# jianzongwu/betrayed-by-captions

Hardware: NVIDIA B200
Metric: decoder_head_images_per_sec_1024 (higher is better)
Workload: dtype bf16

## Files before the change

### betrayed-by-captions_b200/csrc/attention_tc.cu

```cuda
#include <cstdio>
#include <cuda_fp16.h>
#include "kernels.h"
#include "tc_ptx.cuh"
#include "tc_state.h"

namespace cgg {

namespace {

constexpr int AT_THREADS = 64 + 512;
constexpr int AT_KT = 128;
constexpr int AT_STAGES = 4;
constexpr int AT_KV_TILE_BYTES = AT_KT * 64;
constexpr int AT_STAGE_BYTES = 4 * AT_KV_TILE_BYTES;
constexpr int AT_Q_BYTES = 128 * 64;
constexpr int AT_P_BYTES = 128 * AT_KT * 2;
constexpr float LOG2E = 1.4426950408889634f;

struct AttnP {
  const float* q; float* out; __nv_bfloat16* out_bf16;
  const uint32_t* bitmap; const uint8_t* all_masked; const uint8_t* live;
  int Q, K, heads, W32, ntiles, nqt;
  int trace;
  int has_r, r_col0, r_lo_off;
  int out_hl;
  int dbg;
};


__device__ __forceinline__ void store_attn_out(const AttnP& p, int b, int qi, int h, int C, const float* o, float inv) {
  if (p.out) {
    float4* dst = reinterpret_cast<float4*>(p.out + ((long)b * p.Q + qi) * C + h * 32);
#pragma unroll
    for (int i = 0; i < 8; ++i)
      dst[i] = make_float4(o[4 * i] * inv, o[4 * i + 1] * inv, o[4 * i + 2] * inv, o[4 * i + 3] * inv);
  }
  if (p.out_bf16) {
    const long ld = p.out_hl == 1 ? 2 * C : C;
    uint4* dst = reinterpret_cast<uint4*>(p.out_bf16 + ((long)b * p.Q + qi) * ld + h * 32);
    uint4* dst_lo = reinterpret_cast<uint4*>(p.out_bf16 + ((long)b * p.Q + qi) * ld + C + h * 32);
#pragma unroll
    for (int i = 0; i < 4; ++i) {
      uint4 pk, pl;
      uint32_t* w = reinterpret_cast<uint32_t*>(&pk);
      uint32_t* wl = reinterpret_cast<uint32_t*>(&pl);
#pragma unroll
      for (int j = 0; j < 4; ++j) {
        const float a0 = o[8 * i + 2 * j] * inv, a1 = o[8 * i + 2 * j + 1] * inv;
        if (p.out_hl == 2) {
          const __half2 h2 = __floats2half2_rn(a0, a1);
          w[j] = *reinterpret_cast<const uint32_t*>(&h2);
        } else {
          __nv_bfloat162 v2 = __floats2bfloat162_rn(a0, a1);
          w[j] = *reinterpret_cast<uint32_t*>(&v2);
          const float2 back = __bfloat1622float2(v2);
          __nv_bfloat162 l2 = __floats2bfloat162_rn(a0 - back.x, a1 - back.y);
          wl[j] = *reinterpret_cast<uint32_t*>(&l2);
        }
      }
      dst[i] = pk;
      if (p.out_hl == 1) dst_lo[i] = pl;
    }
  }
}

__device__ __forceinline__ void tmem_ld32(uint32_t taddr, float* v) {
  uint32_t r[32];
  asm volatile(
      "tcgen05.ld.sync.aligned.32x32b.x32.b32 {%0, %1, %2, %3, %4, %5, %6, %7, %8, %9, %10, %11, %12, %13, %14, %15, "
      "%16, %17, %18, %19, %20, %21, %22, %23, %24, %25, %26, %27, %28, %29, %30, %31}, [%32];"
      : "=r"(r[0]), "=r"(r[1]), "=r"(r[2]), "=r"(r[3]), "=r"(r[4]), "=r"(r[5]), "=r"(r[6]), "=r"(r[7]), "=r"(r[8]),
        "=r"(r[9]), "=r"(r[10]), "=r"(r[11]), "=r"(r[12]), "=r"(r[13]), "=r"(r[14]), "=r"(r[15]), "=r"(r[16]),
        "=r"(r[17]), "=r"(r[18]), "=r"(r[19]), "=r"(r[20]), "=r"(r[21]), "=r"(r[22]), "=r"(r[23]), "=r"(r[24]),
        "=r"(r[25]), "=r"(r[26]), "=r"(r[27]), "=r"(r[28]), "=r"(r[29]), "=r"(r[30]), "=r"(r[31])
      : "r"(taddr));
  asm volatile("tcgen05.wait::ld.sync.aligned;" ::: "memory");
#pragma unroll
  for (int i = 0; i < 32; ++i) v[i] = __uint_as_float(r[i]);
}

__device__ __forceinline__ float fast_exp2(float x) {
  float y;
  asm("ex2.approx.ftz.f32 %0, %1;" : "=f"(y) : "f"(x));
  return y;
}

__device__ __forceinline__ uint64_t umma_desc(uint32_t addr, uint32_t lbo, uint32_t sbo, uint32_t layout) {
  return (uint64_t)((addr >> 4) & 0x3FFFu) | ((uint64_t)((lbo >> 4) & 0x3FFFu) << 16) |
         ((uint64_t)((sbo >> 4) & 0x3FFFu) << 32) | (1ull << 46) | ((uint64_t)layout << 61);
}

__device__ __forceinline__ void fence_async_smem() { asm volatile("fence.proxy.async.shared::cta;" ::: "memory"); }

__device__ __forceinline__ int next_live(const uint8_t* live, int t, int n) {
  while (t < n && !live[t]) ++t;
  return t;
}

__device__ long long g_at_trace[64];
#ifdef CGG_AT_TRACING
#define AT_TRACE(ti, slot)                                                                                   \
  do {                                                                                                       \
    if (p.trace && blockIdx.x == 0 && blockIdx.y == 0 && (ti) >= 16 && (ti) < 24) g_at_trace[((ti) - 16) * 8 + (slot)] = clock64(); \
  } while (0)
#define AT_TRACE_W(ti, slot) do { if (warp == p.trace && lane == 0) AT_TRACE(ti, slot); } while (0)
#else
#define AT_TRACE(ti, slot) do { } while (0)
#define AT_TRACE_W(ti, slot) do { } while (0)
#endif

__global__ void __launch_bounds__(AT_THREADS, 1)
attention_tc_kernel(const __grid_constant__ CUtensorMap tmK, const __grid_constant__ CUtensorMap tmV,
                    const __grid_constant__ CUtensorMap tmR, const __grid_constant__ AttnP p) {
  extern __shared__ uint8_t smem_raw[];
  uint8_t* smem = reinterpret_cast<uint8_t*>((reinterpret_cast<uintptr_t>(smem_raw) + 1023) & ~(uintptr_t)1023);
  uint8_t* sQ = smem;
  uint8_t* sP = sQ + AT_Q_BYTES;
  uint8_t* sKV = sP + 2 * AT_P_BYTES;
  uint8_t* sLive = sKV + AT_STAGES * AT_STAGE_BYTES;
  uint64_t* bars = reinterpret_cast<uint64_t*>(sLive + 512);
  uint64_t* kv_full = bars;
  uint64_t* kv_empty = kv_full + AT_STAGES;
  uint64_t* step = kv_empty + AT_STAGES;
  uint64_t* p_full = step + 2;
  uint32_t* tmem_slot = reinterpret_cast<uint32_t*>(p_full + 2);

  const int warp = threadIdx.x >> 5, lane = threadIdx.x & 31;
  const int h = blockIdx.x % p.heads, qt = blockIdx.x / p.heads, b = blockIdx.y;
  const uint8_t* live = sLive;
  const int C = p.heads * 32;

  if (warp == 0 && lane == 0) {
    ptx::prefetch_tmap(&tmK);
    ptx::prefetch_tmap(&tmV);
    if (p.has_r) ptx::prefetch_tmap(&tmR);
    for (int i = 0; i < AT_STAGES; ++i) { ptx::mbar_init(&kv_full[i], 1); ptx::mbar_init(&kv_empty[i], 1); }
    for (int i = 0; i < 2; ++i) { ptx::mbar_init(&step[i], 1); ptx::mbar_init(&p_full[i], 512); }
    ptx::fence_mbar_init();
  }
  if (warp == 1) {
    ptx::tmem_alloc(tmem_slot, 512);
    ptx::tmem_relinquish();
  }
  ptx::grid_dep_launch();
  ptx::grid_dep_wait();
  {
    const int q0 = qt * 128, nrows = min(128, p.Q - q0);
    bool all_live = p.bitmap == nullptr;
    if (!all_live && p.all_masked)
      for (int r = lane; r < nrows; r += 32) all_live = all_live || p.all_masked[(long)b * p.Q + q0 + r] != 0;
    all_live = __any_sync(0xffffffffu, all_live);
    for (int t = warp; t < p.ntiles; t += AT_THREADS / 32) {
      bool any = all_live;
      if (!all_live) {
        for (int r = lane; r < nrows; r += 32) {
          const uint32_t* brow = p.bitmap + ((long)b * p.Q + q0 + r) * p.W32;
#pragma unroll
          for (int w = 0; w < 4; ++w) {
            const int widx = t * 4 + w, k0 = t * AT_KT + w * 32;
            if (widx < p.W32 && k0 < p.K) {
              const uint32_t valid = (k0 + 32 > p.K) ? ((1u << (p.K - k0)) - 1u) : 0xffffffffu;
              any = any || ((~__ldg(brow + widx)) & valid) != 0u;
            }
          }
        }
      }
      any = __any_sync(0xffffffffu, any);
      if (lane == 0) sLive[t] = any ? 1 : 0;
    }
  }
  if (warp >= 2 && warp < 6) {
    const int row = (warp & 3) * 32 + lane, qi = qt * 128 + row;
    float qv[32];
    if (qi < p.Q) {
      const float4* src = reinterpret_cast<const float4*>(p.q + ((long)b * p.Q + qi) * C + h * 32);
#pragma unroll
      for (int i = 0; i < 8; ++i) {
        const float4 x = __ldg(src + i);
        qv[4 * i] = x.x; qv[4 * i + 1] = x.y; qv[4 * i + 2] = x.z; qv[4 * i + 3] = x.w;
      }
    } else {
#pragma unroll
      for (int i = 0; i < 32; ++i) qv[i] = 0.f;
    }
#pragma unroll
    for (int c = 0; c < 4; ++c) {
      uint4 pk;
      uint32_t* w = reinterpret_cast<uint32_t*>(&pk);
#pragma unroll
      for (int j = 0; j < 4; ++j) {
        __nv_bfloat162 v2 = __floats2bfloat162_rn(qv[8 * c + 2 * j], qv[8 * c + 2 * j + 1]);
        w[j] = *reinterpret_cast<uint32_t*>(&v2);
      }
      *reinterpret_cast<uint4*>(sQ + (row >> 3) * 512 + c * 128 + (row & 7) * 16) = pk;
    }
    fence_async_smem();
  }
  ptx::tc_fence_before();
  __syncthreads();
  ptx::tc_fence_after();
  const uint32_t tmem_base = *tmem_slot;
  const uint32_t tmem_S = tmem_base;
  const uint32_t tmem_O = tmem_base + 256;

  if (warp == 0) {
    if (lane == 0) {
      int it = 0;
      for (int t = next_live(live, 0, p.ntiles); t < p.ntiles; t = next_live(live, t + 1, p.ntiles), ++it) {
        const int s = it % AT_STAGES;
        ptx::mbar_wait(&kv_empty[s], ((uint32_t)(it / AT_STAGES) & 1u) ^ 1u);
        ptx::mbar_expect_tx(&kv_full[s], (p.has_r ? (p.has_r > 1 ? 4 : 3) : 2) * AT_KV_TILE_BYTES);
        uint8_t* st = sKV + s * AT_STAGE_BYTES;
        if (p.has_r) {
          ptx::tma_load_2d(st + 2 * AT_KV_TILE_BYTES, &tmR, &kv_full[s], p.r_col0 + h * 32, t * AT_KT);
          if (p.has_r > 1) ptx::tma_load_2d(st + 3 * AT_KV_TILE_BYTES, &tmR, &kv_full[s], p.r_lo_off + p.r_col0 + h * 32, t * AT_KT);
        }
        ptx::tma_load_3d(st, &tmK, &kv_full[s], h * 32, t * AT_KT, b);
        ptx::tma_load_3d(st + AT_KV_TILE_BYTES, &tmV, &kv_full[s], h * 32, t * AT_KT, b);
      }
    }
  } else if (warp == 1) {
    const uint32_t idesc_s = ptx::umma_idesc_bf16(128, AT_KT, false, false);
    const uint32_t idesc_o = ptx::umma_idesc_bf16(128, 32, false, true);
    int n_live = 0;
    for (int t = 0; t < p.ntiles; ++t) n_live += live[t] ? 1 : 0;
    const uint64_t qd0 = umma_desc(ptx::smem_u32(sQ), 128, 512, 0);
    const uint64_t kd0 = umma_desc(ptx::smem_u32(sKV), 16, 512, 4);
    const uint64_t vd0 = umma_desc(ptx::smem_u32(sKV + AT_KV_TILE_BYTES), 1024, 512, 4);
    const uint64_t pd0 = umma_desc(ptx::smem_u32(sP), 128, 2048, 0);
    auto wait_kv = [&](int j) {
      ptx::mbar_wait(&kv_full[j % AT_STAGES], (uint32_t)(j / AT_STAGES) & 1u);
      ptx::tc_fence_after();
    };
    auto issue_qk = [&](int j) {
      const uint64_t kd = kd0 + (uint64_t)((j % AT_STAGES) * (AT_STAGE_BYTES >> 4));
      const uint32_t d = tmem_S + (uint32_t)((j & 1) * 128);
#pragma unroll
      for (int k = 0; k < 2; ++k) ptx::mma_bf16_ss(d, qd0 + (uint64_t)(k * 16), kd + (uint64_t)(k * 2), idesc_s, k);
      if (p.has_r) {
#pragma unroll
        for (int k = 0; k < 4; ++k)
          if (k < 2 || p.has_r > 1)
            ptx::mma_bf16_ss(d, qd0 + (uint64_t)((k & 1) * 16),
                             kd + (uint64_t)((((2 + (k >> 1)) * AT_KV_TILE_BYTES) >> 4) + (k & 1) * 2), idesc_s, 1u);
      }
    };
    for (int j = 0; j < 2 && j < n_live; ++j) {
      wait_kv(j);
      if (ptx::elect_one()) { issue_qk(j); ptx::mma_commit(&step[j]); }
      __syncwarp();
    }
    for (int j = 0; j < n_live; ++j) {
      const int s = j % AT_STAGES;
      ptx::mbar_wait(&p_full[j & 1], (uint32_t)(j >> 1) & 1u);
      if (j + 2 < n_live) wait_kv(j + 2);
      ptx::tc_fence_after();
      if (lane == 0) AT_TRACE(j, 0);
      if (ptx::elect_one()) {
        const uint64_t pd = pd0 + (uint64_t)((j & 1) * (AT_P_BYTES >> 4));
        const uint64_t vd = vd0 + (uint64_t)(s * (AT_STAGE_BYTES >> 4));
#pragma unroll
        for (int cq = 0; cq < 4; ++cq) {
#pragma unroll
          for (int k = 0; k < 2; ++k)
            ptx::mma_bf16_ss(tmem_O + (uint32_t)(((j & 1) * 4 + cq) * 32), pd + (uint64_t)((cq * 512 + k * 256) >> 4),
                             vd + (uint64_t)((cq * 2048 + k * 1024) >> 4), idesc_o, k);
        }
        if (j + 2 < n_live) issue_qk(j + 2);
        ptx::mma_commit(&step[j & 1]);
      }
      __syncwarp();
      if (lane == 0) AT_TRACE(j, 2);
    }
  } else {
    const int quarter = warp & 3;
    const int cq = (warp - 2) >> 2;
    const int row = quarter * 32 + lane, qi = qt * 128 + row;
    const bool row_ok = qi < p.Q;
    const uint32_t lane_off = (uint32_t)(quarter * 32) << 16;
    const bool ignore_mask = !row_ok || p.bitmap == nullptr || (p.all_masked && p.all_masked[(long)b * p.Q + qi]);
    const uint32_t* brow = p.bitmap ? p.bitmap + ((long)b * p.Q + (row_ok ? qi : 0)) * p.W32 : nullptr;
    float m_run = -INFINITY, l_run = 0.f;
    float o[32];
#pragma unroll
    for (int i = 0; i < 32; ++i) o[i] = 0.f;
    auto fold_o = [&](int pb, float scale) {
      float ov[32];
      tmem_ld32(tmem_O + (uint32_t)((pb * 4 + cq) * 32) + lane_off, ov);
      if (__all_sync(0xffffffffu, scale == 1.f)) {
#pragma unroll
        for (int i = 0; i < 32; ++i) o[i] += ov[i];
      } else {
#pragma unroll
        for (int i = 0; i < 32; ++i) o[i] = (o[i] + ov[i]) * scale;
      }
    };
    auto load_mask = [&](int t) -> uint32_t {
      const int widx = t * 4 + cq;
      uint32_t word = 0u;
      if (!ignore_mask && widx < p.W32) word = __ldg(brow + widx);
      const int k0 = t * AT_KT + cq * 32;
      if (k0 + 32 > p.K) word |= (k0 >= p.K) ? 0xffffffffu : ~((1u << (p.K - k0)) - 1u);
      return word;
    };
    int it = 0;
    uint32_t mw_next = 0u;
    {
      const int t0 = next_live(live, 0, p.ntiles);
      if (t0 < p.ntiles) mw_next = load_mask(t0);
    }
    for (int t = next_live(live, 0, p.ntiles); t < p.ntiles; ++it) {
      const int buf = it & 1;
      const int t_next = next_live(live, t + 1, p.ntiles);
      const uint32_t mw = mw_next;
      if (t_next < p.ntiles) mw_next = load_mask(t_next);
      ptx::mbar_wait(&step[buf], (uint32_t)(it >> 1) & 1u);
      ptx::tc_fence_after();
      AT_TRACE_W(it, 3);
      float v[32];
      tmem_ld32(tmem_S + (uint32_t)(buf * 128 + cq * 32) + lane_off, v);
      AT_TRACE_W(it, 4);
      float mx = -INFINITY;
#pragma unroll
      for (int i = 0; i < 32; ++i) {
        if ((mw >> i) & 1u) v[i] = -INFINITY;
        mx = fmaxf(mx, v[i]);
      }
      const float m_new = fmaxf(m_run, mx);
      const float scale = (m_new == -INFINITY) ? 1.f : fast_exp2((m_run - m_new) * LOG2E);
      const float mneg = (m_new == -INFINITY) ? 0.f : -m_new * LOG2E;
      m_run = m_new;
      uint8_t* prow = sP + buf * AT_P_BYTES + (row >> 3) * 2048 + (row & 7) * 16 + cq * 512;
      float psum = 0.f;
#pragma unroll
      for (int g = 0; g < 4; ++g) {
        uint4 pk;
        uint32_t* w = reinterpret_cast<uint32_t*>(&pk);
#pragma unroll
        for (int j = 0; j < 4; ++j) {
          const int i0 = g * 8 + 2 * j;
          const float e0 = fast_exp2(fmaf(v[i0], LOG2E, mneg)), e1 = fast_exp2(fmaf(v[i0 + 1], LOG2E, mneg));
          __nv_bfloat162 v2 = __floats2bfloat162_rn(e0, e1);
          w[j] = *reinterpret_cast<uint32_t*>(&v2);
          psum += e0 + e1;
        }
        *reinterpret_cast<uint4*>(prow + g * 128) = pk;
      }
      l_run = l_run * scale + psum;
      fence_async_smem();
      ptx::tc_fence_before();
      ptx::mbar_arrive(&p_full[buf]);
      AT_TRACE_W(it, 5);
      if (it > 0) {
        ptx::mbar_wait(&step[(it - 1) & 1], (uint32_t)(((it - 1) >> 1) + 1) & 1u);
        ptx::tc_fence_after();
        if (warp == 2 && lane == 0) ptx::mbar_arrive(&kv_empty[(it - 1) % AT_STAGES]);
        AT_TRACE_W(it, 6);
        fold_o((it - 1) & 1, scale);
      }
      AT_TRACE_W(it, 7);
      t = t_next;
    }
    if (it > 0) {
      ptx::mbar_wait(&step[(it - 1) & 1], (uint32_t)(((it - 1) >> 1) + 1) & 1u);
      ptx::tc_fence_after();
      fold_o((it - 1) & 1, 1.f);
    }
    float* xch = reinterpret_cast<float*>(sP);
    if (cq > 0) {
      float* dst = xch + ((cq - 1) * 128 + row) * 35;
      dst[0] = m_run;
      dst[1] = l_run;
#pragma unroll
      for (int i = 0; i < 32; ++i) dst[2 + i] = o[i];
    }
    asm volatile("bar.sync 1, 512;" ::: "memory");
    const int hf = cq;
    if (cq == 0) {
      float m = m_run;
#pragma unroll
      for (int c2 = 0; c2 < 3; ++c2) m = fmaxf(m, xch[(c2 * 128 + row) * 35]);
      const float a0 = (m_run == -INFINITY) ? 0.f : fast_exp2((m_run - m) * LOG2E);
      l_run *= a0;
#pragma unroll
      for (int i = 0; i < 32; ++i) o[i] *= a0;
#pragma unroll
      for (int c2 = 0; c2 < 3; ++c2) {
        const float* src = xch + (c2 * 128 + row) * 35;
        const float m1 = src[0];
        const float a1 = (m1 == -INFINITY) ? 0.f : fast_exp2((m1 - m) * LOG2E);
        l_run += src[1] * a1;
#pragma unroll
        for (int i = 0; i < 32; ++i) o[i] += src[2 + i] * a1;
      }
    }
    if (row_ok && hf == 0) store_attn_out(p, b, qi, h, C, o, l_run > 0.f ? 1.0f / l_run : 0.f);
  }
  ptx::tc_fence_before();
  __syncthreads();
  if (warp == 1) {
    __syncwarp();
    ptx::tmem_dealloc(tmem_base, 512);
  }
}


__device__ __forceinline__ void tmem_st32(uint32_t taddr, const float* v) {
  asm volatile(
      "tcgen05.st.sync.aligned.32x32b.x32.b32 [%0], {%1, %2, %3, %4, %5, %6, %7, %8, %9, %10, %11, %12, %13, %14, %15, %16, "
      "%17, %18, %19, %20, %21, %22, %23, %24, %25, %26, %27, %28, %29, %30, %31, %32};"
      ::"r"(taddr), "r"(__float_as_uint(v[0])), "r"(__float_as_uint(v[1])), "r"(__float_as_uint(v[2])), "r"(__float_as_uint(v[3])),
        "r"(__float_as_uint(v[4])), "r"(__float_as_uint(v[5])), "r"(__float_as_uint(v[6])), "r"(__float_as_uint(v[7])),
        "r"(__float_as_uint(v[8])), "r"(__float_as_uint(v[9])), "r"(__float_as_uint(v[10])), "r"(__float_as_uint(v[11])),
        "r"(__float_as_uint(v[12])), "r"(__float_as_uint(v[13])), "r"(__float_as_uint(v[14])), "r"(__float_as_uint(v[15])),
        "r"(__float_as_uint(v[16])), "r"(__float_as_uint(v[17])), "r"(__float_as_uint(v[18])), "r"(__float_as_uint(v[19])),
        "r"(__float_as_uint(v[20])), "r"(__float_as_uint(v[21])), "r"(__float_as_uint(v[22])), "r"(__float_as_uint(v[23])),
        "r"(__float_as_uint(v[24])), "r"(__float_as_uint(v[25])), "r"(__float_as_uint(v[26])), "r"(__float_as_uint(v[27])),
        "r"(__float_as_uint(v[28])), "r"(__float_as_uint(v[29])), "r"(__float_as_uint(v[30])), "r"(__float_as_uint(v[31]))
      : "memory");
  asm volatile("tcgen05.wait::st.sync.aligned;" ::: "memory");
}
__device__ __forceinline__ void tmem_st16(uint32_t taddr, const uint32_t* r) {
  asm volatile(
      "tcgen05.st.sync.aligned.32x32b.x16.b32 [%0], {%1, %2, %3, %4, %5, %6, %7, %8, %9, %10, %11, %12, %13, %14, %15, %16};"
      ::"r"(taddr), "r"(r[0]), "r"(r[1]), "r"(r[2]), "r"(r[3]), "r"(r[4]), "r"(r[5]), "r"(r[6]), "r"(r[7]), "r"(r[8]), "r"(r[9]),
        "r"(r[10]), "r"(r[11]), "r"(r[12]), "r"(r[13]), "r"(r[14]), "r"(r[15])
      : "memory");
  asm volatile("tcgen05.wait::st.sync.aligned;" ::: "memory");
}
__device__ __forceinline__ void mma_bf16_ts(uint32_t d_tmem, uint32_t a_tmem, uint64_t bdesc, uint32_t idesc, uint32_t accumulate) {
  asm volatile(
      "{\n\t.reg .pred p;\n\tsetp.ne.b32 p, %4, 0;\n\t"
      "tcgen05.mma.cta_group::1.kind::f16 [%0], [%1], %2, %3, p;\n\t}\n"
      ::"r"(d_tmem), "r"(a_tmem), "l"(bdesc), "r"(idesc), "r"(accumulate)
      : "memory");
}

constexpr float AT2_TAU = 8.0f;

__global__ void __launch_bounds__(AT_THREADS, 1)
attention_tc2_kernel(const __grid_constant__ CUtensorMap tmK, const __grid_constant__ CUtensorMap tmV,
                     const __grid_constant__ CUtensorMap tmR, const __grid_constant__ AttnP p) {
  extern __shared__ uint8_t smem_raw[];
  uint8_t* smem = reinterpret_cast<uint8_t*>((reinterpret_cast<uintptr_t>(smem_raw) + 1023) & ~(uintptr_t)1023);
  uint8_t* sQ = smem;
  uint8_t* sX = sQ + AT_Q_BYTES;
  uint8_t* sKV = sX + 2 * AT_P_BYTES;
  uint8_t* sLive = sKV + AT_STAGES * AT_STAGE_BYTES;
  uint64_t* bars = reinterpret_cast<uint64_t*>(sLive + 512);
  uint64_t* kv_full = bars;
  uint64_t* kv_empty = kv_full + AT_STAGES;
  uint64_t* step = kv_empty + AT_STAGES;
  uint64_t* p_full = step + 2;
  uint32_t* tmem_slot = reinterpret_cast<uint32_t*>(p_full + 2);

  const int warp = threadIdx.x >> 5, lane = threadIdx.x & 31;
  const int h = blockIdx.x % p.heads, qt = blockIdx.x / p.heads, b = blockIdx.y;
  const uint8_t* live = sLive;
  const int C = p.heads * 32;

  if (warp == 0 && lane == 0) {
    ptx::prefetch_tmap(&tmK);
    ptx::prefetch_tmap(&tmV);
    if (p.has_r) ptx::prefetch_tmap(&tmR);
    for (int i = 0; i < AT_STAGES; ++i) { ptx::mbar_init(&kv_full[i], 1); ptx::mbar_init(&kv_empty[i], 1); }
    for (int i = 0; i < 2; ++i) { ptx::mbar_init(&step[i], 1); ptx::mbar_init(&p_full[i], 512); }
    ptx::fence_mbar_init();
  }
  if (warp == 1) {
    ptx::tmem_alloc(tmem_slot, 512);
    ptx::tmem_relinquish();
  }
  ptx::grid_dep_launch();
  ptx::grid_dep_wait();
  {
    const int q0 = qt * 128, nrows = min(128, p.Q - q0);
    bool all_live = p.bitmap == nullptr;
    if (!all_live && p.all_masked)
      for (int r = lane; r < nrows; r += 32) all_live = all_live || p.all_masked[(long)b * p.Q + q0 + r] != 0;
    all_live = __any_sync(0xffffffffu, all_live);
    for (int t = warp; t < p.ntiles; t += AT_THREADS / 32) {
      bool any = all_live;
      if (!all_live) {
        for (int r = lane; r < nrows; r += 32) {
          const uint32_t* brow = p.bitmap + ((long)b * p.Q + q0 + r) * p.W32;
#pragma unroll
          for (int w = 0; w < 4; ++w) {
            const int widx = t * 4 + w, k0 = t * AT_KT + w * 32;
            if (widx < p.W32 && k0 < p.K) {
              const uint32_t valid = (k0 + 32 > p.K) ? ((1u << (p.K - k0)) - 1u) : 0xffffffffu;
              any = any || ((~__ldg(brow + widx)) & valid) != 0u;
            }
          }
        }
      }
      any = __any_sync(0xffffffffu, any);
      if (lane == 0) sLive[t] = any ? 1 : 0;
    }
  }
  if (warp >= 2 && warp < 6) {
    const int row = (warp & 3) * 32 + lane, qi = qt * 128 + row;
    float qv[32];
    if (qi < p.Q) {
      const float4* src = reinterpret_cast<const float4*>(p.q + ((long)b * p.Q + qi) * C + h * 32);
#pragma unroll
      for (int i = 0; i < 8; ++i) {
        const float4 x = __ldg(src + i);
        qv[4 * i] = x.x; qv[4 * i + 1] = x.y; qv[4 * i + 2] = x.z; qv[4 * i + 3] = x.w;
      }
    } else {
#pragma unroll
      for (int i = 0; i < 32; ++i) qv[i] = 0.f;
    }
#pragma unroll
    for (int c = 0; c < 4; ++c) {
      uint4 pk;
      uint32_t* w = reinterpret_cast<uint32_t*>(&pk);
#pragma unroll
      for (int j = 0; j < 4; ++j) {
        __nv_bfloat162 v2 = __floats2bfloat162_rn(qv[8 * c + 2 * j], qv[8 * c + 2 * j + 1]);
        w[j] = *reinterpret_cast<uint32_t*>(&v2);
      }
      *reinterpret_cast<uint4*>(sQ + (row >> 3) * 512 + c * 128 + (row & 7) * 16) = pk;
    }
    fence_async_smem();
  }
  ptx::tc_fence_before();
  __syncthreads();
  ptx::tc_fence_after();
  const uint32_t tmem_base = *tmem_slot;
  const uint32_t tmem_S = tmem_base;
  const uint32_t tmem_P = tmem_base + 256;
  const uint32_t tmem_O = tmem_base + 384;

  if (warp == 0) {
    if (lane == 0) {
      int it = 0;
      for (int t = next_live(live, 0, p.ntiles); t < p.ntiles; t = next_live(live, t + 1, p.ntiles), ++it) {
        const int s = it % AT_STAGES;
        ptx::mbar_wait(&kv_empty[s], ((uint32_t)(it / AT_STAGES) & 1u) ^ 1u);
        ptx::mbar_expect_tx(&kv_full[s], (p.has_r ? (p.has_r > 1 ? 4 : 3) : 2) * AT_KV_TILE_BYTES);
        uint8_t* st = sKV + s * AT_STAGE_BYTES;
        if (p.has_r) {
          ptx::tma_load_2d(st + 2 * AT_KV_TILE_BYTES, &tmR, &kv_full[s], p.r_col0 + h * 32, t * AT_KT);
          if (p.has_r > 1) ptx::tma_load_2d(st + 3 * AT_KV_TILE_BYTES, &tmR, &kv_full[s], p.r_lo_off + p.r_col0 + h * 32, t * AT_KT);
        }
        ptx::tma_load_3d(st, &tmK, &kv_full[s], h * 32, t * AT_KT, b);
        ptx::tma_load_3d(st + AT_KV_TILE_BYTES, &tmV, &kv_full[s], h * 32, t * AT_KT, b);
      }
    }
  } else if (warp == 1) {
    const uint32_t idesc_s = ptx::umma_idesc_bf16(128, AT_KT, false, false);
    const uint32_t idesc_o = ptx::umma_idesc_bf16(128, 32, false, true);
    int n_live = 0;
    for (int t = 0; t < p.ntiles; ++t) n_live += live[t] ? 1 : 0;
    const uint64_t qd0 = umma_desc(ptx::smem_u32(sQ), 128, 512, 0);
    const uint64_t kd0 = umma_desc(ptx::smem_u32(sKV), 16, 512, 4);
    const uint64_t vd0 = umma_desc(ptx::smem_u32(sKV + AT_KV_TILE_BYTES), 1024, 512, 4);
    auto wait_kv = [&](int j) {
      ptx::mbar_wait(&kv_full[j % AT_STAGES], (uint32_t)(j / AT_STAGES) & 1u);
      ptx::tc_fence_after();
    };
    auto issue_qk = [&](int j) {
      const uint64_t kd = kd0 + (uint64_t)((j % AT_STAGES) * (AT_STAGE_BYTES >> 4));
      const uint32_t d = tmem_S + (uint32_t)((j & 1) * 128);
#pragma unroll
      for (int k = 0; k < 2; ++k) ptx::mma_bf16_ss(d, qd0 + (uint64_t)(k * 16), kd + (uint64_t)(k * 2), idesc_s, k);
      if (p.has_r) {
#pragma unroll
        for (int k = 0; k < 4; ++k)
          if (k < 2 || p.has_r > 1)
            ptx::mma_bf16_ss(d, qd0 + (uint64_t)((k & 1) * 16),
                             kd + (uint64_t)((((2 + (k >> 1)) * AT_KV_TILE_BYTES) >> 4) + (k & 1) * 2), idesc_s, 1u);
      }
    };
    for (int j = 0; j < 2 && j < n_live; ++j) {
      wait_kv(j);
      if (ptx::elect_one()) { issue_qk(j); ptx::mma_commit(&step[j]); }
      __syncwarp();
    }
    for (int j = 0; j < n_live; ++j) {
      const int s = j % AT_STAGES;
      ptx::mbar_wait(&p_full[j & 1], (uint32_t)(j >> 1) & 1u);
      if (lane == 0) AT_TRACE(j, 0);
      if (j + 2 < n_live) wait_kv(j + 2);
      ptx::tc_fence_after();
      if (lane == 0) AT_TRACE(j, 1);
      if (ptx::elect_one()) {
        const uint64_t vd = vd0 + (uint64_t)(s * (AT_STAGE_BYTES >> 4));
        const uint32_t pa = tmem_P + (uint32_t)((j & 1) * 64);
#pragma unroll
        for (int cq = 0; cq < 4; ++cq) {
          if (p.dbg & 2) break;
#pragma unroll
          for (int k = 0; k < 2; ++k)
            mma_bf16_ts(tmem_O + (uint32_t)(cq * 32), pa + (uint32_t)(cq * 16 + k * 8),
                        vd + (uint64_t)((cq * 2048 + k * 1024) >> 4), idesc_o, (j > 0 || k > 0) ? 1u : 0u);
        }
        if (j + 2 < n_live) issue_qk(j + 2);
        ptx::mma_commit(&step[j & 1]);
      }
      __syncwarp();
      if (lane == 0) AT_TRACE(j, 2);
    }
  } else {
    const int quarter = warp & 3;
    const int cq = (warp - 2) >> 2;
    const int row = quarter * 32 + lane, qi = qt * 128 + row;
    const bool row_ok = qi < p.Q;
    const uint32_t lane_off = (uint32_t)(quarter * 32) << 16;
    const bool ignore_mask = !row_ok || p.bitmap == nullptr || (p.all_masked && p.all_masked[(long)b * p.Q + qi]);
    const uint32_t* brow = p.bitmap ? p.bitmap + ((long)b * p.Q + (row_ok ? qi : 0)) * p.W32 : nullptr;
    const uint32_t taddr_o = tmem_O + (uint32_t)(cq * 32) + lane_off;
    float m_ref = -INFINITY, l_run = 0.f;
    auto load_mask = [&](int t) -> uint32_t {
      const int widx = t * 4 + cq;
      uint32_t word = 0u;
      if (!ignore_mask && widx < p.W32) word = __ldg(brow + widx);
      const int k0 = t * AT_KT + cq * 32;
      if (k0 + 32 > p.K) word |= (k0 >= p.K) ? 0xffffffffu : ~((1u << (p.K - k0)) - 1u);
      return word;
    };
    int it = 0;
    uint32_t mw_next = 0u;
    {
      const int t0 = next_live(live, 0, p.ntiles);
      if (t0 < p.ntiles) mw_next = load_mask(t0);
    }
    for (int t = next_live(live, 0, p.ntiles); t < p.ntiles; ++it) {
      const int buf = it & 1;
      const int t_next = next_live(live, t + 1, p.ntiles);
      const uint32_t mw = mw_next;
      if (t_next < p.ntiles) mw_next = load_mask(t_next);
      ptx::mbar_wait(&step[buf], (uint32_t)(it >> 1) & 1u);
      ptx::tc_fence_after();
      AT_TRACE_W(it, 3);
      float v[32];
      tmem_ld32(tmem_S + (uint32_t)(buf * 128 + cq * 32) + lane_off, v);
      AT_TRACE_W(it, 4);
      float mx = -INFINITY;
#pragma unroll
      for (int i = 0; i < 32; ++i) {
        if ((mw >> i) & 1u) v[i] = -INFINITY;
        mx = fmaxf(mx, v[i]);
      }
      mx *= LOG2E;
      const bool move = mx > m_ref + AT2_TAU;
      const bool fix = move && m_ref != -INFINITY;
      if (__any_sync(0xffffffffu, fix)) {
        ptx::mbar_wait(&step[(it - 1) & 1], (uint32_t)(((it - 1) >> 1) + 1) & 1u);
        ptx::tc_fence_after();
        const float sc = fix ? fast_exp2(m_ref - mx) : 1.f;
        float ov[32];
        tmem_ld32(taddr_o, ov);
#pragma unroll
        for (int i = 0; i < 32; ++i) ov[i] *= sc;
        tmem_st32(taddr_o, ov);
        l_run *= sc;
      }
      if (move) m_ref = mx;
      AT_TRACE_W(it, 5);
      const float mneg = (m_ref == -INFINITY) ? 0.f : -m_ref;
      uint32_t pk[16];
      float psum = 0.f;
#pragma unroll
      for (int j = 0; j < 16; ++j) {
        float e0, e1;
        if (p.dbg & 4) { e0 = fmaf(v[2 * j], LOG2E, mneg); e1 = fmaf(v[2 * j + 1], LOG2E, mneg); }
        else { e0 = fast_exp2(fmaf(v[2 * j], LOG2E, mneg)); e1 = fast_exp2(fmaf(v[2 * j + 1], LOG2E, mneg)); }
        __nv_bfloat162 v2 = __floats2bfloat162_rn(e0, e1);
        pk[j] = *reinterpret_cast<uint32_t*>(&v2);
        psum += e0 + e1;
      }
      l_run += psum;
      AT_TRACE_W(it, 6);
      tmem_st16(tmem_P + (uint32_t)(buf * 64 + cq * 16) + lane_off, pk);
      ptx::tc_fence_before();
      ptx::mbar_arrive(&p_full[buf]);
      AT_TRACE_W(it, 7);
      if (it > 0 && warp == 2) {
        ptx::mbar_wait(&step[(it - 1) & 1], (uint32_t)(((it - 1) >> 1) + 1) & 1u);
        if (lane == 0) ptx::mbar_arrive(&kv_empty[(it - 1) % AT_STAGES]);
      }
      t = t_next;
    }
    float o[32];
    if (it > 0) {
      ptx::mbar_wait(&step[(it - 1) & 1], (uint32_t)(((it - 1) >> 1) + 1) & 1u);
      ptx::tc_fence_after();
      tmem_ld32(taddr_o, o);
    } else {
#pragma unroll
      for (int i = 0; i < 32; ++i) o[i] = 0.f;
    }
    float* xch = reinterpret_cast<float*>(sX);
    if (cq > 0) {
      float* dst = xch + ((cq - 1) * 128 + row) * 35;
      dst[0] = m_ref;
      dst[1] = l_run;
#pragma unroll
      for (int i = 0; i < 32; ++i) dst[2 + i] = o[i];
    }
    asm volatile("bar.sync 1, 512;" ::: "memory");
    if (cq == 0) {
      float m = m_ref;
#pragma unroll
      for (int c2 = 0; c2 < 3; ++c2) m = fmaxf(m, xch[(c2 * 128 + row) * 35]);
      const float a0 = (m_ref == -INFINITY) ? 0.f : fast_exp2(m_ref - m);
      l_run *= a0;
#pragma unroll
      for (int i = 0; i < 32; ++i) o[i] = (m_ref == -INFINITY) ? 0.f : o[i] * a0;
#pragma unroll
      for (int c2 = 0; c2 < 3; ++c2) {
        const float* src = xch + (c2 * 128 + row) * 35;
        const float m1 = src[0];
        if (m1 != -INFINITY) {
          const float a1 = fast_exp2(m1 - m);
          l_run += src[1] * a1;
#pragma unroll
          for (int i = 0; i < 32; ++i) o[i] += src[2 + i] * a1;
        }
      }
      if (row_ok) store_attn_out(p, b, qi, h, C, o, l_run > 0.f ? 1.0f / l_run : 0.f);
    }
  }
  ptx::tc_fence_before();
  __syncthreads();
  if (warp == 1) {
    __syncwarp();
    ptx::tmem_dealloc(tmem_base, 512);
  }
}

constexpr int AT3_STAGES = 6;

__global__ void __launch_bounds__(AT_THREADS, 1)
attention_tc3_kernel(const __grid_constant__ CUtensorMap tmK, const __grid_constant__ CUtensorMap tmV,
                     const __grid_constant__ CUtensorMap tmR, const __grid_constant__ AttnP p) {
  extern __shared__ uint8_t smem_raw[];
  uint8_t* smem = reinterpret_cast<uint8_t*>((reinterpret_cast<uintptr_t>(smem_raw) + 1023) & ~(uintptr_t)1023);
  uint8_t* sQ = smem;
  uint8_t* sKV = sQ + AT_Q_BYTES;
  uint8_t* sX = sKV;
  uint8_t* sLive = sKV + AT3_STAGES * AT_STAGE_BYTES;
  uint64_t* bars = reinterpret_cast<uint64_t*>(sLive + 512);
  uint64_t* kv_full = bars;
  uint64_t* kv_empty = kv_full + AT3_STAGES;
  uint64_t* step = kv_empty + AT3_STAGES;
  uint64_t* p_full = step + 3;
  uint32_t* tmem_slot = reinterpret_cast<uint32_t*>(p_full + 3);

  const int warp = threadIdx.x >> 5, lane = threadIdx.x & 31;
  const int h = blockIdx.x % p.heads, qt = blockIdx.x / p.heads, b = blockIdx.y;
  const uint8_t* live = sLive;
  const int C = p.heads * 32;

  if (warp == 0 && lane == 0) {
    ptx::prefetch_tmap(&tmK);
    ptx::prefetch_tmap(&tmV);
    if (p.has_r) ptx::prefetch_tmap(&tmR);
    for (int i = 0; i < AT3_STAGES; ++i) { ptx::mbar_init(&kv_full[i], 1); ptx::mbar_init(&kv_empty[i], 1); }
    for (int i = 0; i < 3; ++i) { ptx::mbar_init(&step[i], 1); ptx::mbar_init(&p_full[i], 512); }
    ptx::fence_mbar_init();
  }
  if (warp == 1) {
    ptx::tmem_alloc(tmem_slot, 512);
    ptx::tmem_relinquish();
  }
  ptx::grid_dep_launch();
  ptx::grid_dep_wait();
  {
    const int q0 = qt * 128, nrows = min(128, p.Q - q0);
    bool all_live = p.bitmap == nullptr;
    if (!all_live && p.all_masked)
      for (int r = lane; r < nrows; r += 32) all_live = all_live || p.all_masked[(long)b * p.Q + q0 + r] != 0;
    all_live = __any_sync(0xffffffffu, all_live);
    for (int t = warp; t < p.ntiles; t += AT_THREADS / 32) {
      bool any = all_live;
      if (!all_live) {
        for (int r = lane; r < nrows; r += 32) {
          const uint32_t* brow = p.bitmap + ((long)b * p.Q + q0 + r) * p.W32;
#pragma unroll
          for (int w = 0; w < 4; ++w) {
            const int widx = t * 4 + w, k0 = t * AT_KT + w * 32;
            if (widx < p.W32 && k0 < p.K) {
              const uint32_t valid = (k0 + 32 > p.K) ? ((1u << (p.K - k0)) - 1u) : 0xffffffffu;
              any = any || ((~__ldg(brow + widx)) & valid) != 0u;
            }
          }
        }
      }
      any = __any_sync(0xffffffffu, any);
      if (lane == 0) sLive[t] = any ? 1 : 0;
    }
  }
  if (warp >= 2 && warp < 6) {
    const int row = (warp & 3) * 32 + lane, qi = qt * 128 + row;
    float qv[32];
    if (qi < p.Q) {
      const float4* src = reinterpret_cast<const float4*>(p.q + ((long)b * p.Q + qi) * C + h * 32);
#pragma unroll
      for (int i = 0; i < 8; ++i) {
        const float4 x = __ldg(src + i);
        qv[4 * i] = x.x; qv[4 * i + 1] = x.y; qv[4 * i + 2] = x.z; qv[4 * i + 3] = x.w;
      }
    } else {
#pragma unroll
      for (int i = 0; i < 32; ++i) qv[i] = 0.f;
    }
#pragma unroll
    for (int c = 0; c < 4; ++c) {
      uint4 pk;
      uint32_t* w = reinterpret_cast<uint32_t*>(&pk);
#pragma unroll
      for (int j = 0; j < 4; ++j) {
        __nv_bfloat162 v2 = __floats2bfloat162_rn(qv[8 * c + 2 * j], qv[8 * c + 2 * j + 1]);
        w[j] = *reinterpret_cast<uint32_t*>(&v2);
      }
      *reinterpret_cast<uint4*>(sQ + (row >> 3) * 512 + c * 128 + (row & 7) * 16) = pk;
    }
    fence_async_smem();
  }
  ptx::tc_fence_before();
  __syncthreads();
  ptx::tc_fence_after();
  const uint32_t tmem_base = *tmem_slot;
  const uint32_t tmem_S = tmem_base;
  const uint32_t tmem_O = tmem_base + 384;

  if (warp == 0) {
    if (lane == 0) {
      int it = 0;
      for (int t = next_live(live, 0, p.ntiles); t < p.ntiles; t = next_live(live, t + 1, p.ntiles), ++it) {
        const int s = it % AT3_STAGES;
        ptx::mbar_wait(&kv_empty[s], ((uint32_t)(it / AT3_STAGES) & 1u) ^ 1u);
        ptx::mbar_expect_tx(&kv_full[s], (p.has_r ? (p.has_r > 1 ? 4 : 3) : 2) * AT_KV_TILE_BYTES);
        uint8_t* st = sKV + s * AT_STAGE_BYTES;
        if (p.has_r) {
          ptx::tma_load_2d(st + 2 * AT_KV_TILE_BYTES, &tmR, &kv_full[s], p.r_col0 + h * 32, t * AT_KT);
          if (p.has_r > 1) ptx::tma_load_2d(st + 3 * AT_KV_TILE_BYTES, &tmR, &kv_full[s], p.r_lo_off + p.r_col0 + h * 32, t * AT_KT);
        }
        ptx::tma_load_3d(st, &tmK, &kv_full[s], h * 32, t * AT_KT, b);
        ptx::tma_load_3d(st + AT_KV_TILE_BYTES, &tmV, &kv_full[s], h * 32, t * AT_KT, b);
      }
    }
  } else if (warp == 1) {
    const uint32_t idesc_s = ptx::umma_idesc_bf16(128, AT_KT, false, false);
    const uint32_t idesc_o = ptx::umma_idesc_bf16(128, 32, false, true);
    int n_live = 0;
    for (int t = 0; t < p.ntiles; ++t) n_live += live[t] ? 1 : 0;
    const uint64_t qd0 = umma_desc(ptx::smem_u32(sQ), 128, 512, 0);
    const uint64_t kd0 = umma_desc(ptx::smem_u32(sKV), 16, 512, 4);
    const uint64_t vd0 = umma_desc(ptx::smem_u32(sKV + AT_KV_TILE_BYTES), 1024, 512, 4);
    auto wait_kv = [&](int j) {
      ptx::mbar_wait(&kv_full[j % AT3_STAGES], (uint32_t)(j / AT3_STAGES) & 1u);
      ptx::tc_fence_after();
    };
    auto issue_qk = [&](int j) {
      const uint64_t kd = kd0 + (uint64_t)((j % AT3_STAGES) * (AT_STAGE_BYTES >> 4));
      const uint32_t d = tmem_S + (uint32_t)((j % 3) * 128);
#pragma unroll
      for (int k = 0; k < 2; ++k) ptx::mma_bf16_ss(d, qd0 + (uint64_t)(k * 16), kd + (uint64_t)(k * 2), idesc_s, k);
      if (p.has_r) {
#pragma unroll
        for (int k = 0; k < 4; ++k)
          if (k < 2 || p.has_r > 1)
            ptx::mma_bf16_ss(d, qd0 + (uint64_t)((k & 1) * 16),
                             kd + (uint64_t)((((2 + (k >> 1)) * AT_KV_TILE_BYTES) >> 4) + (k & 1) * 2), idesc_s, 1u);
      }
    };
    for (int j = 0; j < 3 && j < n_live; ++j) {
      wait_kv(j);
      if (ptx::elect_one()) { issue_qk(j); ptx::mma_commit(&step[j]); }
      __syncwarp();
    }
    for (int j = 0; j < n_live; ++j) {
      const int s = j % AT3_STAGES;
      ptx::mbar_wait(&p_full[j % 3], (uint32_t)(j / 3) & 1u);
      if (lane == 0) AT_TRACE(j, 0);
      if (j + 3 < n_live) wait_kv(j + 3);
      ptx::tc_fence_after();
      if (lane == 0) AT_TRACE(j, 1);
      if (ptx::elect_one()) {
        const uint64_t vd = vd0 + (uint64_t)(s * (AT_STAGE_BYTES >> 4));
        const uint32_t pa = tmem_S + (uint32_t)((j % 3) * 128);
#pragma unroll
        for (int cq = 0; cq < 4; ++cq) {
          if (p.dbg & 2) break;
#pragma unroll
          for (int k = 0; k < 2; ++k)
            mma_bf16_ts(tmem_O + (uint32_t)(cq * 32), pa + (uint32_t)(cq * 32 + k * 8),
                        vd + (uint64_t)((cq * 2048 + k * 1024) >> 4), idesc_o, (j > 0 || k > 0) ? 1u : 0u);
        }
        if (j + 3 < n_live) issue_qk(j + 3);
        ptx::mma_commit(&step[j % 3]);
      }
      __syncwarp();
      if (lane == 0) AT_TRACE(j, 2);
    }
  } else {
    const int quarter = warp & 3;
    const int cq = (warp - 2) >> 2;
    const int row = quarter * 32 + lane, qi = qt * 128 + row;
    const bool row_ok = qi < p.Q;
    const uint32_t lane_off = (uint32_t)(quarter * 32) << 16;
    const bool ignore_mask = !row_ok || p.bitmap == nullptr || (p.all_masked && p.all_masked[(long)b * p.Q + qi]);
    const uint32_t* brow = p.bitmap ? p.bitmap + ((long)b * p.Q + (row_ok ? qi : 0)) * p.W32 : nullptr;
    const uint32_t taddr_o = tmem_O + (uint32_t)(cq * 32) + lane_off;
    float m_ref = -INFINITY, l_run = 0.f;
    auto load_mask = [&](int t) -> uint32_t {
      const int widx = t * 4 + cq;
      uint32_t word = 0u;
      if (!ignore_mask && widx < p.W32) word = __ldg(brow + widx);
      const int k0 = t * AT_KT + cq * 32;
      if (k0 + 32 > p.K) word |= (k0 >= p.K) ? 0xffffffffu : ~((1u << (p.K - k0)) - 1u);
      return word;
    };
    int it = 0;
    uint32_t mw_next = 0u;
    {
      const int t0 = next_live(live, 0, p.ntiles);
      if (t0 < p.ntiles) mw_next = load_mask(t0);
    }
    for (int t = next_live(live, 0, p.ntiles); t < p.ntiles; ++it) {
      const int buf = it % 3;
      const int t_next = next_live(live, t + 1, p.ntiles);
      const uint32_t mw = mw_next;
      if (t_next < p.ntiles) mw_next = load_mask(t_next);
      ptx::mbar_wait(&step[buf], (uint32_t)(it / 3) & 1u);
      ptx::tc_fence_after();
      AT_TRACE_W(it, 3);
      float v[32];
      tmem_ld32(tmem_S + (uint32_t)(buf * 128 + cq * 32) + lane_off, v);
      AT_TRACE_W(it, 4);
      float mx = -INFINITY;
#pragma unroll
      for (int i = 0; i < 32; ++i) {
        if ((mw >> i) & 1u) v[i] = -INFINITY;
        mx = fmaxf(mx, v[i]);
      }
      mx *= LOG2E;
      const bool move = mx > m_ref + AT2_TAU;
      const bool fix = move && m_ref != -INFINITY;
      if (__any_sync(0xffffffffu, fix)) {
        ptx::mbar_wait(&step[(it - 1) % 3], (uint32_t)(((it - 1) / 3) + 1) & 1u);
        ptx::tc_fence_after();
        const float sc = fix ? fast_exp2(m_ref - mx) : 1.f;
        float ov[32];
        tmem_ld32(taddr_o, ov);
#pragma unroll
        for (int i = 0; i < 32; ++i) ov[i] *= sc;
        tmem_st32(taddr_o, ov);
        l_run *= sc;
      }
      if (move) m_ref = mx;
      AT_TRACE_W(it, 5);
      const float mneg = (m_ref == -INFINITY) ? 0.f : -m_ref;
      uint32_t pk[16];
      float psum = 0.f;
#pragma unroll
      for (int j = 0; j < 16; ++j) {
        float e0, e1;
        if (p.dbg & 4) { e0 = fmaf(v[2 * j], LOG2E, mneg); e1 = fmaf(v[2 * j + 1], LOG2E, mneg); }
        else { e0 = fast_exp2(fmaf(v[2 * j], LOG2E, mneg)); e1 = fast_exp2(fmaf(v[2 * j + 1], LOG2E, mneg)); }
        __nv_bfloat162 v2 = __floats2bfloat162_rn(e0, e1);
        pk[j] = *reinterpret_cast<uint32_t*>(&v2);
        psum += e0 + e1;
      }
      l_run += psum;
      AT_TRACE_W(it, 6);
      tmem_st16(tmem_S + (uint32_t)(buf * 128 + cq * 32) + lane_off, pk);
      ptx::tc_fence_before();
      ptx::mbar_arrive(&p_full[buf]);
      AT_TRACE_W(it, 7);
      if (it > 0 && warp == 2) {
        ptx::mbar_wait(&step[(it - 1) % 3], (uint32_t)(((it - 1) / 3) + 1) & 1u);
        if (lane == 0) ptx::mbar_arrive(&kv_empty[(it - 1) % AT3_STAGES]);
      }
      t = t_next;
    }
    float o[32];
    if (it > 0) {
      ptx::mbar_wait(&step[(it - 1) % 3], (uint32_t)(((it - 1) / 3) + 1) & 1u);
      ptx::tc_fence_after();
      tmem_ld32(taddr_o, o);
    } else {
#pragma unroll
      for (int i = 0; i < 32; ++i) o[i] = 0.f;
    }
    asm volatile("bar.sync 1, 512;" ::: "memory");
    float* xch = reinterpret_cast<float*>(sX);
    if (cq > 0) {
      float* dst = xch + ((cq - 1) * 128 + row) * 35;
      dst[0] = m_ref;
      dst[1] = l_run;
#pragma unroll
      for (int i = 0; i < 32; ++i) dst[2 + i] = o[i];
    }
    asm volatile("bar.sync 1, 512;" ::: "memory");
    if (cq == 0) {
      float m = m_ref;
#pragma unroll
      for (int c2 = 0; c2 < 3; ++c2) m = fmaxf(m, xch[(c2 * 128 + row) * 35]);
      const float a0 = (m_ref == -INFINITY) ? 0.f : fast_exp2(m_ref - m);
      l_run *= a0;
#pragma unroll
      for (int i = 0; i < 32; ++i) o[i] = (m_ref == -INFINITY) ? 0.f : o[i] * a0;
#pragma unroll
      for (int c2 = 0; c2 < 3; ++c2) {
        const float* src = xch + (c2 * 128 + row) * 35;
        const float m1 = src[0];
        if (m1 != -INFINITY) {
          const float a1 = fast_exp2(m1 - m);
          l_run += src[1] * a1;
#pragma unroll
          for (int i = 0; i < 32; ++i) o[i] += src[2 + i] * a1;
        }
      }
      if (row_ok) store_attn_out(p, b, qi, h, C, o, l_run > 0.f ? 1.0f / l_run : 0.f);
    }
  }
  ptx::tc_fence_before();
  __syncthreads();
  if (warp == 1) {
    __syncwarp();
    ptx::tmem_dealloc(tmem_base, 512);
  }
}

int make_map_kv(TcState* t, CUtensorMap* m, const void* base, int K, long kv_stride, long kv_bstride, int B, int C) {
  if ((kv_stride * 2) % 16 != 0 || (kv_bstride * 2) % 16 != 0 || (reinterpret_cast<uintptr_t>(base) & 15))
    return tc_fail(t, CGG_ERR_UNSUPPORTED, "K/V rows must be 16-byte aligned");
  cuuint64_t dims[3] = {(cuuint64_t)C, (cuuint64_t)K, (cuuint64_t)B};
  cuuint64_t strides[2] = {(cuuint64_t)kv_stride * 2, (cuuint64_t)kv_bstride * 2};
  cuuint32_t box[3] = {32, AT_KT, 1};
  cuuint32_t es[3] = {1, 1, 1};
  CUresult r = t->encode(m, CU_TENSOR_MAP_DATA_TYPE_BFLOAT16, 3, const_cast<void*>(base), dims, strides, box, es,
                         CU_TENSOR_MAP_INTERLEAVE_NONE, CU_TENSOR_MAP_SWIZZLE_64B, CU_TENSOR_MAP_L2_PROMOTION_L2_128B,
                         CU_TENSOR_MAP_FLOAT_OOB_FILL_NONE);
  if (r != CUDA_SUCCESS) return tc_fail(t, CGG_ERR_CUDA, "cuTensorMapEncodeTiled(KV) failed: " + std::to_string((int)r));
  return CGG_OK;
}

}

int tc_attention(TcState* t, int batch, int num_keys, const float* q, const void* k, const void* v, long kv_stride,
                 long kv_bstride, const uint32_t* bitmap, const uint8_t* all_masked, float* out, __nv_bfloat16* out_bf16,
                 cudaStream_t s, const void* r_table, long r_cols, int r_col0, int out_mode) {
  const int Q = t->cfg.num_queries, heads = t->cfg.num_heads, C = t->cfg.embed_dim;
  const int ntiles = (num_keys + AT_KT - 1) / AT_KT, nqt = (Q + 127) / 128;
  CUtensorMap mK, mV;
  int st = make_map_kv(t, &mK, k, num_keys, kv_stride, kv_bstride, batch, C);
  if (st != CGG_OK) return st;
  st = make_map_kv(t, &mV, v, num_keys, kv_stride, kv_bstride, batch, C);
  if (st != CGG_OK) return st;
  CUtensorMap mR = mK;
  if (r_table) {
    cuuint64_t dims[2] = {(cuuint64_t)r_cols, (cuuint64_t)num_keys};
    cuuint64_t strides[1] = {(cuuint64_t)r_cols * 2};
    cuuint32_t box[2] = {32, AT_KT};
    cuuint32_t es[2] = {1, 1};
    CUresult r = t->encode(&mR, CU_TENSOR_MAP_DATA_TYPE_BFLOAT16, 2, const_cast<void*>(r_table), dims, strides, box, es,
                           CU_TENSOR_MAP_INTERLEAVE_NONE, CU_TENSOR_MAP_SWIZZLE_64B, CU_TENSOR_MAP_L2_PROMOTION_L2_128B,
                           CU_TENSOR_MAP_FLOAT_OOB_FILL_NONE);
    if (r != CUDA_SUCCESS) return tc_fail(t, CGG_ERR_CUDA, "cuTensorMapEncodeTiled(R) failed: " + std::to_string((int)r));
  }
  const int W32 = (num_keys + 31) / 32;
  AttnP p;
  p.q = q; p.out = out; p.out_bf16 = out_bf16; p.bitmap = bitmap; p.all_masked = all_masked; p.live = nullptr;
  p.Q = Q; p.K = num_keys; p.heads = heads; p.W32 = W32; p.ntiles = ntiles; p.nqt = nqt;
  p.has_r = r_table ? 2 : 0;
  p.r_col0 = r_col0; p.r_lo_off = (int)(r_cols / 2);
  p.out_hl = out_mode;
#ifdef CGG_AT_TRACING
  static const int at_dbg = getenv("CGG_AT_DBG") ? atoi(getenv("CGG_AT_DBG")) : 0;
  p.dbg = at_dbg;
  if (at_dbg & 1) p.has_r = 0;
#else
  p.dbg = 0;
#endif
  if (ntiles > 512) return tc_fail(t, CGG_ERR_BAD_SHAPE, "more than 512 key tiles");
  const size_t smem = 1024 + AT_Q_BYTES + 2 * AT_P_BYTES + AT_STAGES * AT_STAGE_BYTES + 512 + (2 * AT_STAGES + 4) * 8 + 16;
  if (!t->attn_attr_set) {
    TCU(cudaFuncSetAttribute(attention_tc_kernel, cudaFuncAttributeMaxDynamicSharedMemorySize, (int)smem));
    TCU(cudaFuncSetAttribute(attention_tc2_kernel, cudaFuncAttributeMaxDynamicSharedMemorySize, (int)smem));
    TCU(cudaFuncSetAttribute(attention_tc3_kernel, cudaFuncAttributeMaxDynamicSharedMemorySize, 227 * 1024));
    t->attn_attr_set = true;
  }
  static const bool trace = getenv("CGG_AT_TRACE") != nullptr;
  p.trace = trace ? atoi(getenv("CGG_AT_TRACE")) : 0;
  static const int use_v1 = getenv("CGG_ATTN_V1") ? atoi(getenv("CGG_ATTN_V1")) : 0;
  static const int use_v3 = getenv("CGG_ATTN_V3") ? atoi(getenv("CGG_ATTN_V3")) : 1;
  const size_t smem3 = 1024 + AT_Q_BYTES + AT3_STAGES * AT_STAGE_BYTES + 512 + (2 * AT3_STAGES + 6) * 8 + 16;
  if (use_v1) TCU(launch_pdl(attention_tc_kernel, dim3(heads * nqt, batch), dim3(AT_THREADS), smem, s, mK, mV, mR, p));
  else if (use_v3) TCU(launch_pdl(attention_tc3_kernel, dim3(heads * nqt, batch), dim3(AT_THREADS), smem3, s, mK, mV, mR, p));
  else TCU(launch_pdl(attention_tc2_kernel, dim3(heads * nqt, batch), dim3(AT_THREADS), smem, s, mK, mV, mR, p));
  count_launch();
  TCU(cudaGetLastError());
  if (trace && ntiles >= 24) {
    cudaStreamSynchronize(s);
    long long tr[64];
    cudaMemcpyFromSymbol(tr, g_at_trace, sizeof(tr));
    fprintf(stderr, "[attention trace] K=%d cycles rel. to tile 16: mma(P ready, PV committed, QK(j+2) committed) softmax(S ready, S loaded, P arrived, O(j-1) ready, folded)\n", num_keys);
    for (int i = 0; i < 8; ++i) {
      fprintf(stderr, "  j=%d:", 16 + i);
      for (int j = 0; j < 8; ++j) fprintf(stderr, " %7lld", tr[i * 8 + j] - tr[0]);
      fprintf(stderr, "\n");
    }
  }
  return CGG_OK;
}

}
```

Baseline: 6497.

## Consolidate masked attention into one kernel with staged masks and precomputed live tiles

Removes the v1/v2 attention variants and keeps a single v3-style kernel. The per-CTA live-tile scan moves into a separate small pre-kernel that writes live flags to global memory. The producer warp now loads the per-row mask words alongside each K/V stage into shared memory, so softmax warps no longer issue their own global mask loads. Other changes: stages go from 4 to 6, TMEM loads and stores are split into issue and wait so they overlap with math, and the max and sum reductions use trees and packed f32x2 math. The cost is an extra kernel launch and a more complex producer path with 32-arrival barriers.

New measurement: 6716 (median of 6 runs). 3.4% higher.

```diff
diff --git a/betrayed-by-captions_b200/csrc/attention_tc.cu b/betrayed-by-captions_b200/csrc/attention_tc.cu
--- a/betrayed-by-captions_b200/csrc/attention_tc.cu
+++ b/betrayed-by-captions_b200/csrc/attention_tc.cu
@@ -10,21 +10,26 @@
 
 constexpr int AT_THREADS = 64 + 512;
 constexpr int AT_KT = 128;
-constexpr int AT_STAGES = 4;
+constexpr int AT_STAGES = 6;
 constexpr int AT_KV_TILE_BYTES = AT_KT * 64;
 constexpr int AT_STAGE_BYTES = 4 * AT_KV_TILE_BYTES;
+constexpr int AT_MASK_BYTES = 128 * 4 * 4;
 constexpr int AT_Q_BYTES = 128 * 64;
-constexpr int AT_P_BYTES = 128 * AT_KT * 2;
+constexpr int AT_MAX_TILES = 512;
 constexpr float LOG2E = 1.4426950408889634f;
+constexpr float AT_TAU = 8.0f;
+constexpr size_t AT_SMEM = 1024 + AT_Q_BYTES + AT_STAGES * (AT_STAGE_BYTES + AT_MASK_BYTES) + AT_MAX_TILES +
+                           (2 * AT_STAGES + 6) * 8 + 16;
+static_assert(AT_SMEM <= 227 * 1024, "attention stage budget");
 
 struct AttnP {
   const float* q; float* out; __nv_bfloat16* out_bf16;
-  const uint32_t* bitmap; const uint8_t* all_masked; const uint8_t* live;
+  const uint32_t* bitmap; const uint8_t* all_masked;
+  const uint8_t* live;
   int Q, K, heads, W32, ntiles, nqt;
   int trace;
   int has_r, r_col0, r_lo_off;
   int out_hl;
-  int dbg;
 };
 
 
@@ -97,6 +102,60 @@
   return t;
 }
 
+__device__ __forceinline__ void tmem_ld32_issue(uint32_t taddr, uint32_t* r) {
+  asm volatile(
+      "tcgen05.ld.sync.aligned.32x32b.x32.b32 {%0, %1, %2, %3, %4, %5, %6, %7, %8, %9, %10, %11, %12, %13, %14, %15, "
+      "%16, %17, %18, %19, %20, %21, %22, %23, %24, %25, %26, %27, %28, %29, %30, %31}, [%32];"
+      : "=r"(r[0]), "=r"(r[1]), "=r"(r[2]), "=r"(r[3]), "=r"(r[4]), "=r"(r[5]), "=r"(r[6]), "=r"(r[7]), "=r"(r[8]),
+        "=r"(r[9]), "=r"(r[10]), "=r"(r[11]), "=r"(r[12]), "=r"(r[13]), "=r"(r[14]), "=r"(r[15]), "=r"(r[16]),
+        "=r"(r[17]), "=r"(r[18]), "=r"(r[19]), "=r"(r[20]), "=r"(r[21]), "=r"(r[22]), "=r"(r[23]), "=r"(r[24]),
+        "=r"(r[25]), "=r"(r[26]), "=r"(r[27]), "=r"(r[28]), "=r"(r[29]), "=r"(r[30]), "=r"(r[31])
+      : "r"(taddr));
+}
+__device__ __forceinline__ void tmem_ld32_wait(uint32_t* r) {
+  asm volatile("tcgen05.wait::ld.sync.aligned;"
+               : "+r"(r[0]), "+r"(r[1]), "+r"(r[2]), "+r"(r[3]), "+r"(r[4]), "+r"(r[5]), "+r"(r[6]), "+r"(r[7]),
+                 "+r"(r[8]), "+r"(r[9]), "+r"(r[10]), "+r"(r[11]), "+r"(r[12]), "+r"(r[13]), "+r"(r[14]), "+r"(r[15]),
+                 "+r"(r[16]), "+r"(r[17]), "+r"(r[18]), "+r"(r[19]), "+r"(r[20]), "+r"(r[21]), "+r"(r[22]),
+                 "+r"(r[23]), "+r"(r[24]), "+r"(r[25]), "+r"(r[26]), "+r"(r[27]), "+r"(r[28]), "+r"(r[29]),
+                 "+r"(r[30]), "+r"(r[31])
+               :: "memory");
+}
+__device__ __forceinline__ void tmem_st16_issue(uint32_t taddr, const uint32_t* r) {
+  asm volatile(
+      "tcgen05.st.sync.aligned.32x32b.x16.b32 [%0], {%1, %2, %3, %4, %5, %6, %7, %8, %9, %10, %11, %12, %13, %14, %15, %16};"
+      ::"r"(taddr), "r"(r[0]), "r"(r[1]), "r"(r[2]), "r"(r[3]), "r"(r[4]), "r"(r[5]), "r"(r[6]), "r"(r[7]), "r"(r[8]), "r"(r[9]),
+        "r"(r[10]), "r"(r[11]), "r"(r[12]), "r"(r[13]), "r"(r[14]), "r"(r[15])
+      : "memory");
+}
+__device__ __forceinline__ void tmem_st16_wait(uint32_t* r) {
+  asm volatile("tcgen05.wait::st.sync.aligned;"
+               : "+r"(r[0]), "+r"(r[1]), "+r"(r[2]), "+r"(r[3]), "+r"(r[4]), "+r"(r[5]), "+r"(r[6]), "+r"(r[7]),
+                 "+r"(r[8]), "+r"(r[9]), "+r"(r[10]), "+r"(r[11]), "+r"(r[12]), "+r"(r[13]), "+r"(r[14]), "+r"(r[15])
+               :: "memory");
+}
+
+__device__ __forceinline__ float2 fma2(float2 a, float2 b, float2 c) {
+  float2 d;
+  asm("{\n\t.reg .b64 ra, rb, rc, rd;\n\t"
+      "mov.b64 ra, {%2, %3};\n\tmov.b64 rb, {%4, %5};\n\tmov.b64 rc, {%6, %7};\n\t"
+      "fma.rn.f32x2 rd, ra, rb, rc;\n\tmov.b64 {%0, %1}, rd;\n\t}"
+      : "=f"(d.x), "=f"(d.y) : "f"(a.x), "f"(a.y), "f"(b.x), "f"(b.y), "f"(c.x), "f"(c.y));
+  return d;
+}
+__device__ __forceinline__ float2 add2(float2 a, float2 b) {
+  float2 d;
+  asm("{\n\t.reg .b64 ra, rb, rd;\n\t"
+      "mov.b64 ra, {%2, %3};\n\tmov.b64 rb, {%4, %5};\n\t"
+      "add.rn.f32x2 rd, ra, rb;\n\tmov.b64 {%0, %1}, rd;\n\t}"
+      : "=f"(d.x), "=f"(d.y) : "f"(a.x), "f"(a.y), "f"(b.x), "f"(b.y));
+  return d;
+}
+
+__device__ __forceinline__ void mbar_expect_tx_only(uint64_t* bar, uint32_t bytes) {
+  asm volatile("mbarrier.expect_tx.relaxed.cta.shared::cta.b64 [%0], %1;" ::"r"(ptx::smem_u32(bar)), "r"(bytes) : "memory");
+}
+
 __device__ long long g_at_trace[64];
 #ifdef CGG_AT_TRACING
 #define AT_TRACE(ti, slot)                                                                                   \
@@ -109,21 +168,58 @@
 #define AT_TRACE_W(ti, slot) do { } while (0)
 #endif
 
+__device__ __forceinline__ void mma_bf16_ts(uint32_t d_tmem, uint32_t a_tmem, uint64_t bdesc, uint32_t idesc, uint32_t accumulate) {
+  asm volatile(
+      "{\n\t.reg .pred p;\n\tsetp.ne.b32 p, %4, 0;\n\t"
+      "tcgen05.mma.cta_group::1.kind::f16 [%0], [%1], %2, %3, p;\n\t}\n"
+      ::"r"(d_tmem), "r"(a_tmem), "l"(bdesc), "r"(idesc), "r"(accumulate)
+      : "memory");
+}
+
+__global__ void __launch_bounds__(512) attention_live_kernel(const uint32_t* __restrict__ bitmap,
+                                                             const uint8_t* __restrict__ all_masked, int Q, int K,
+                                                             int W32, int ntiles, int nqt, uint8_t* __restrict__ live) {
+  __shared__ int s_tile[AT_MAX_TILES];
+  __shared__ int s_fallback;
+  const int qt = blockIdx.x, b = blockIdx.y, warp = threadIdx.x >> 5, lane = threadIdx.x & 31;
+  for (int t = threadIdx.x; t < ntiles; t += blockDim.x) s_tile[t] = 0;
+  if (threadIdx.x == 0) s_fallback = 0;
+  ptx::grid_dep_launch();
+  ptx::grid_dep_wait();
+  __syncthreads();
+  const int q0 = qt * 128, nrows = min(128, Q - q0);
+  for (int r = warp; r < nrows; r += blockDim.x / 32) {
+    const long row = (long)b * Q + q0 + r;
+    if (all_masked && all_masked[row]) { s_fallback = 1; continue; }
+    const uint32_t* brow = bitmap + row * W32;
+#pragma unroll 4
+    for (int w = lane; w < W32; w += 32) {
+      const int k0 = w * 32;
+      const uint32_t valid = (k0 + 32 > K) ? ((1u << (K - k0)) - 1u) : 0xffffffffu;
+      if ((~__ldg(brow + w)) & valid) s_tile[w >> 2] = 1;
+    }
+  }
+  __syncthreads();
+  for (int t = threadIdx.x; t < ntiles; t += blockDim.x)
+    live[((long)b * nqt + qt) * ntiles + t] = (s_fallback || s_tile[t]) ? 1 : 0;
+}
+
 __global__ void __launch_bounds__(AT_THREADS, 1)
-attention_tc_kernel(const __grid_constant__ CUtensorMap tmK, const __grid_constant__ CUtensorMap tmV,
-                    const __grid_constant__ CUtensorMap tmR, const __grid_constant__ AttnP p) {
+masked_attention_tc_kernel(const __grid_constant__ CUtensorMap tmK, const __grid_constant__ CUtensorMap tmV,
+                           const __grid_constant__ CUtensorMap tmR, const __grid_constant__ AttnP p) {
   extern __shared__ uint8_t smem_raw[];
   uint8_t* smem = reinterpret_cast<uint8_t*>((reinterpret_cast<uintptr_t>(smem_raw) + 1023) & ~(uintptr_t)1023);
   uint8_t* sQ = smem;
-  uint8_t* sP = sQ + AT_Q_BYTES;
-  uint8_t* sKV = sP + 2 * AT_P_BYTES;
-  uint8_t* sLive = sKV + AT_STAGES * AT_STAGE_BYTES;
-  uint64_t* bars = reinterpret_cast<uint64_t*>(sLive + 512);
+  uint8_t* sKV = sQ + AT_Q_BYTES;
+  uint8_t* sX = sKV;
+  uint32_t* sMask = reinterpret_cast<uint32_t*>(sKV + AT_STAGES * AT_STAGE_BYTES);
+  uint8_t* sLive = reinterpret_cast<uint8_t*>(sMask) + AT_STAGES * AT_MASK_BYTES;
+  uint64_t* bars = reinterpret_cast<uint64_t*>(sLive + AT_MAX_TILES);
   uint64_t* kv_full = bars;
   uint64_t* kv_empty = kv_full + AT_STAGES;
   uint64_t* step = kv_empty + AT_STAGES;
-  uint64_t* p_full = step + 2;
-  uint32_t* tmem_slot = reinterpret_cast<uint32_t*>(p_full + 2);
+  uint64_t* p_full = step + 3;
+  uint32_t* tmem_slot = reinterpret_cast<uint32_t*>(p_full + 3);
 
   const int warp = threadIdx.x >> 5, lane = threadIdx.x & 31;
   const int h = blockIdx.x % p.heads, qt = blockIdx.x / p.heads, b = blockIdx.y;
@@ -134,8 +230,8 @@
     ptx::prefetch_tmap(&tmK);
     ptx::prefetch_tmap(&tmV);
     if (p.has_r) ptx::prefetch_tmap(&tmR);
-    for (int i = 0; i < AT_STAGES; ++i) { ptx::mbar_init(&kv_full[i], 1); ptx::mbar_init(&kv_empty[i], 1); }
-    for (int i = 0; i < 2; ++i) { ptx::mbar_init(&step[i], 1); ptx::mbar_init(&p_full[i], 512); }
+    for (int i = 0; i < AT_STAGES; ++i) { ptx::mbar_init(&kv_full[i], 32); ptx::mbar_init(&kv_empty[i], 1); }
+    for (int i = 0; i < 3; ++i) { ptx::mbar_init(&step[i], 1); ptx::mbar_init(&p_full[i], 512); }
     ptx::fence_mbar_init();
   }
   if (warp == 1) {
@@ -145,29 +241,8 @@
   ptx::grid_dep_launch();
   ptx::grid_dep_wait();
   {
-    const int q0 = qt * 128, nrows = min(128, p.Q - q0);
-    bool all_live = p.bitmap == nullptr;
-    if (!all_live && p.all_masked)
-      for (int r = lane; r < nrows; r += 32) all_live = all_live || p.all_masked[(long)b * p.Q + q0 + r] != 0;
-    all_live = __any_sync(0xffffffffu, all_live);
-    for (int t = warp; t < p.ntiles; t += AT_THREADS / 32) {
-      bool any = all_live;
-      if (!all_live) {
-        for (int r = lane; r < nrows; r += 32) {
-          const uint32_t* brow = p.bitmap + ((long)b * p.Q + q0 + r) * p.W32;
-#pragma unroll
-          for (int w = 0; w < 4; ++w) {
-            const int widx = t * 4 + w, k0 = t * AT_KT + w * 32;
-            if (widx < p.W32 && k0 < p.K) {
-              const uint32_t valid = (k0 + 32 > p.K) ? ((1u << (p.K - k0)) - 1u) : 0xffffffffu;
-              any = any || ((~__ldg(brow + widx)) & valid) != 0u;
-            }
-          }
-        }
-      }
-      any = __any_sync(0xffffffffu, any);
-      if (lane == 0) sLive[t] = any ? 1 : 0;
-    }
+    const uint8_t* src = p.live ? p.live + ((long)b * p.nqt + qt) * p.ntiles : nullptr;
+    for (int t = threadIdx.x; t < p.ntiles; t += AT_THREADS) sLive[t] = src ? src[t] : 1;
   }
   if (warp >= 2 && warp < 6) {
     const int row = (warp & 3) * 32 + lane, qi = qt * 128 + row;
@@ -201,15 +276,24 @@
   ptx::tc_fence_after();
   const uint32_t tmem_base = *tmem_slot;
   const uint32_t tmem_S = tmem_base;
-  const uint32_t tmem_O = tmem_base + 256;
+  const uint32_t tmem_O = tmem_base + 384;
 
   if (warp == 0) {
-    if (lane == 0) {
-      int it = 0;
-      for (int t = next_live(live, 0, p.ntiles); t < p.ntiles; t = next_live(live, t + 1, p.ntiles), ++it) {
-        const int s = it % AT_STAGES;
-        ptx::mbar_wait(&kv_empty[s], ((uint32_t)(it / AT_STAGES) & 1u) ^ 1u);
-        ptx::mbar_expect_tx(&kv_full[s], (p.has_r ? (p.has_r > 1 ? 4 : 3) : 2) * AT_KV_TILE_BYTES);
+    const uint32_t* brow[4];
+#pragma unroll
+    for (int i = 0; i < 4; ++i) {
+      const int qi = qt * 128 + lane + 32 * i;
+      const bool use = p.bitmap && qi < p.Q && !(p.all_masked && p.all_masked[(long)b * p.Q + qi]);
+      brow[i] = use ? p.bitmap + ((long)b * p.Q + qi) * p.W32 : nullptr;
+    }
+    const bool vec = (p.W32 & 3) == 0 && (reinterpret_cast<uintptr_t>(p.bitmap) & 15) == 0;
+    const uint32_t tx_bytes = (p.has_r ? (p.has_r > 1 ? 4 : 3) : 2) * AT_KV_TILE_BYTES;
+    int it = 0;
+    for (int t = next_live(live, 0, p.ntiles); t < p.ntiles; t = next_live(live, t + 1, p.ntiles), ++it) {
+      const int s = it % AT_STAGES;
+      ptx::mbar_wait(&kv_empty[s], ((uint32_t)(it / AT_STAGES) & 1u) ^ 1u);
+      if (lane == 0) {
+        mbar_expect_tx_only(&kv_full[s], tx_bytes);
         uint8_t* st = sKV + s * AT_STAGE_BYTES;
         if (p.has_r) {
           ptx::tma_load_2d(st + 2 * AT_KV_TILE_BYTES, &tmR, &kv_full[s], p.r_col0 + h * 32, t * AT_KT);
@@ -218,336 +302,26 @@
         ptx::tma_load_3d(st, &tmK, &kv_full[s], h * 32, t * AT_KT, b);
         ptx::tma_load_3d(st + AT_KV_TILE_BYTES, &tmV, &kv_full[s], h * 32, t * AT_KT, b);
       }
-    }
-  } else if (warp == 1) {
-    const uint32_t idesc_s = ptx::umma_idesc_bf16(128, AT_KT, false, false);
-    const uint32_t idesc_o = ptx::umma_idesc_bf16(128, 32, false, true);
-    int n_live = 0;
-    for (int t = 0; t < p.ntiles; ++t) n_live += live[t] ? 1 : 0;
-    const uint64_t qd0 = umma_desc(ptx::smem_u32(sQ), 128, 512, 0);
-    const uint64_t kd0 = umma_desc(ptx::smem_u32(sKV), 16, 512, 4);
-    const uint64_t vd0 = umma_desc(ptx::smem_u32(sKV + AT_KV_TILE_BYTES), 1024, 512, 4);
-    const uint64_t pd0 = umma_desc(ptx::smem_u32(sP), 128, 2048, 0);
-    auto wait_kv = [&](int j) {
-      ptx::mbar_wait(&kv_full[j % AT_STAGES], (uint32_t)(j / AT_STAGES) & 1u);
-      ptx::tc_fence_after();
-    };
-    auto issue_qk = [&](int j) {
-      const uint64_t kd = kd0 + (uint64_t)((j % AT_STAGES) * (AT_STAGE_BYTES >> 4));
-      const uint32_t d = tmem_S + (uint32_t)((j & 1) * 128);
-#pragma unroll
-      for (int k = 0; k < 2; ++k) ptx::mma_bf16_ss(d, qd0 + (uint64_t)(k * 16), kd + (uint64_t)(k * 2), idesc_s, k);
-      if (p.has_r) {
-#pragma unroll
-        for (int k = 0; k < 4; ++k)
-          if (k < 2 || p.has_r > 1)
-            ptx::mma_bf16_ss(d, qd0 + (uint64_t)((k & 1) * 16),
-                             kd + (uint64_t)((((2 + (k >> 1)) * AT_KV_TILE_BYTES) >> 4) + (k & 1) * 2), idesc_s, 1u);
-      }
-    };
-    for (int j = 0; j < 2 && j < n_live; ++j) {
-      wait_kv(j);
-      if (ptx::elect_one()) { issue_qk(j); ptx::mma_commit(&step[j]); }
-      __syncwarp();
-    }
-    for (int j = 0; j < n_live; ++j) {
-      const int s = j % AT_STAGES;
-      ptx::mbar_wait(&p_full[j & 1], (uint32_t)(j >> 1) & 1u);
-      if (j + 2 < n_live) wait_kv(j + 2);
-      ptx::tc_fence_after();
-      if (lane == 0) AT_TRACE(j, 0);
-      if (ptx::elect_one()) {
-        const uint64_t pd = pd0 + (uint64_t)((j & 1) * (AT_P_BYTES >> 4));
-        const uint64_t vd = vd0 + (uint64_t)(s * (AT_STAGE_BYTES >> 4));
-#pragma unroll
-        for (int cq = 0; cq < 4; ++cq) {
-#pragma unroll
-          for (int k = 0; k < 2; ++k)
-            ptx::mma_bf16_ss(tmem_O + (uint32_t)(((j & 1) * 4 + cq) * 32), pd + (uint64_t)((cq * 512 + k * 256) >> 4),
-                             vd + (uint64_t)((cq * 2048 + k * 1024) >> 4), idesc_o, k);
+      uint32_t w[4][4];
+#pragma unroll
+      for (int i = 0; i < 4; ++i) {
+        if (brow[i] && vec) {
+          const uint4 x = __ldg(reinterpret_cast<const uint4*>(brow[i] + t * 4));
+          w[i][0] = x.x; w[i][1] = x.y; w[i][2] = x.z; w[i][3] = x.w;
+        } else {
+#pragma unroll
+          for (int c = 0; c < 4; ++c) w[i][c] = (brow[i] && t * 4 + c < p.W32) ? __ldg(brow[i] + t * 4 + c) : 0u;
         }
-        if (j + 2 < n_live) issue_qk(j + 2);
-        ptx::mma_commit(&step[j & 1]);
-      }
-      __syncwarp();
-      if (lane == 0) AT_TRACE(j, 2);
-    }
-  } else {
-    const int quarter = warp & 3;
-    const int cq = (warp - 2) >> 2;
-    const int row = quarter * 32 + lane, qi = qt * 128 + row;
-    const bool row_ok = qi < p.Q;
-    const uint32_t lane_off = (uint32_t)(quarter * 32) << 16;
-    const bool ignore_mask = !row_ok || p.bitmap == nullptr || (p.all_masked && p.all_masked[(long)b * p.Q + qi]);
-    const uint32_t* brow = p.bitmap ? p.bitmap + ((long)b * p.Q + (row_ok ? qi : 0)) * p.W32 : nullptr;
-    float m_run = -INFINITY, l_run = 0.f;
-    float o[32];
-#pragma unroll
-    for (int i = 0; i < 32; ++i) o[i] = 0.f;
-    auto fold_o = [&](int pb, float scale) {
-      float ov[32];
-      tmem_ld32(tmem_O + (uint32_t)((pb * 4 + cq) * 32) + lane_off, ov);
-      if (__all_sync(0xffffffffu, scale == 1.f)) {
-#pragma unroll
-        for (int i = 0; i < 32; ++i) o[i] += ov[i];
-      } else {
-#pragma unroll
-        for (int i = 0; i < 32; ++i) o[i] = (o[i] + ov[i]) * scale;
-      }
-    };
-    auto load_mask = [&](int t) -> uint32_t {
-      const int widx = t * 4 + cq;
-      uint32_t word = 0u;
-      if (!ignore_mask && widx < p.W32) word = __ldg(brow + widx);
-      const int k0 = t * AT_KT + cq * 32;
-      if (k0 + 32 > p.K) word |= (k0 >= p.K) ? 0xffffffffu : ~((1u << (p.K - k0)) - 1u);
-      return word;
-    };
-    int it = 0;
-    uint32_t mw_next = 0u;
-    {
-      const int t0 = next_live(live, 0, p.ntiles);
-      if (t0 < p.ntiles) mw_next = load_mask(t0);
-    }
-    for (int t = next_live(live, 0, p.ntiles); t < p.ntiles; ++it) {
-      const int buf = it & 1;
-      const int t_next = next_live(live, t + 1, p.ntiles);
-      const uint32_t mw = mw_next;
-      if (t_next < p.ntiles) mw_next = load_mask(t_next);
-      ptx::mbar_wait(&step[buf], (uint32_t)(it >> 1) & 1u);
-      ptx::tc_fence_after();
-      AT_TRACE_W(it, 3);
-      float v[32];
-      tmem_ld32(tmem_S + (uint32_t)(buf * 128 + cq * 32) + lane_off, v);
-      AT_TRACE_W(it, 4);
-      float mx = -INFINITY;
-#pragma unroll
-      for (int i = 0; i < 32; ++i) {
-        if ((mw >> i) & 1u) v[i] = -INFINITY;
-        mx = fmaxf(mx, v[i]);
-      }
-      const float m_new = fmaxf(m_run, mx);
-      const float scale = (m_new == -INFINITY) ? 1.f : fast_exp2((m_run - m_new) * LOG2E);
-      const float mneg = (m_new == -INFINITY) ? 0.f : -m_new * LOG2E;
-      m_run = m_new;
-      uint8_t* prow = sP + buf * AT_P_BYTES + (row >> 3) * 2048 + (row & 7) * 16 + cq * 512;
-      float psum = 0.f;
-#pragma unroll
-      for (int g = 0; g < 4; ++g) {
-        uint4 pk;
-        uint32_t* w = reinterpret_cast<uint32_t*>(&pk);
-#pragma unroll
-        for (int j = 0; j < 4; ++j) {
-          const int i0 = g * 8 + 2 * j;
-          const float e0 = fast_exp2(fmaf(v[i0], LOG2E, mneg)), e1 = fast_exp2(fmaf(v[i0 + 1], LOG2E, mneg));
-          __nv_bfloat162 v2 = __floats2bfloat162_rn(e0, e1);
-          w[j] = *reinterpret_cast<uint32_t*>(&v2);
-          psum += e0 + e1;
-        }
-        *reinterpret_cast<uint4*>(prow + g * 128) = pk;
-      }
-      l_run = l_run * scale + psum;
-      fence_async_smem();
-      ptx::tc_fence_before();
-      ptx::mbar_arrive(&p_full[buf]);
-      AT_TRACE_W(it, 5);
-      if (it > 0) {
-        ptx::mbar_wait(&step[(it - 1) & 1], (uint32_t)(((it - 1) >> 1) + 1) & 1u);
-        ptx::tc_fence_after();
-        if (warp == 2 && lane == 0) ptx::mbar_arrive(&kv_empty[(it - 1) % AT_STAGES]);
-        AT_TRACE_W(it, 6);
-        fold_o((it - 1) & 1, scale);
-      }
-      AT_TRACE_W(it, 7);
-      t = t_next;
-    }
-    if (it > 0) {
-      ptx::mbar_wait(&step[(it - 1) & 1], (uint32_t)(((it - 1) >> 1) + 1) & 1u);
-      ptx::tc_fence_after();
-      fold_o((it - 1) & 1, 1.f);
-    }
-    float* xch = reinterpret_cast<float*>(sP);
-    if (cq > 0) {
-      float* dst = xch + ((cq - 1) * 128 + row) * 35;
-      dst[0] = m_run;
-      dst[1] = l_run;
-#pragma unroll
-      for (int i = 0; i < 32; ++i) dst[2 + i] = o[i];
-    }
-    asm volatile("bar.sync 1, 512;" ::: "memory");
-    const int hf = cq;
-    if (cq == 0) {
-      float m = m_run;
-#pragma unroll
-      for (int c2 = 0; c2 < 3; ++c2) m = fmaxf(m, xch[(c2 * 128 + row) * 35]);
-      const float a0 = (m_run == -INFINITY) ? 0.f : fast_exp2((m_run - m) * LOG2E);
-      l_run *= a0;
-#pragma unroll
-      for (int i = 0; i < 32; ++i) o[i] *= a0;
-#pragma unroll
-      for (int c2 = 0; c2 < 3; ++c2) {
-        const float* src = xch + (c2 * 128 + row) * 35;
-        const float m1 = src[0];
-        const float a1 = (m1 == -INFINITY) ? 0.f : fast_exp2((m1 - m) * LOG2E);
-        l_run += src[1] * a1;
-#pragma unroll
-        for (int i = 0; i < 32; ++i) o[i] += src[2 + i] * a1;
-      }
-    }
-    if (row_ok && hf == 0) store_attn_out(p, b, qi, h, C, o, l_run > 0.f ? 1.0f / l_run : 0.f);
-  }
-  ptx::tc_fence_before();
-  __syncthreads();
-  if (warp == 1) {
-    __syncwarp();
-    ptx::tmem_dealloc(tmem_base, 512);
-  }
-}
-
-
-__device__ __forceinline__ void tmem_st32(uint32_t taddr, const float* v) {
-  asm volatile(
-      "tcgen05.st.sync.aligned.32x32b.x32.b32 [%0], {%1, %2, %3, %4, %5, %6, %7, %8, %9, %10, %11, %12, %13, %14, %15, %16, "
-      "%17, %18, %19, %20, %21, %22, %23, %24, %25, %26, %27, %28, %29, %30, %31, %32};"
-      ::"r"(taddr), "r"(__float_as_uint(v[0])), "r"(__float_as_uint(v[1])), "r"(__float_as_uint(v[2])), "r"(__float_as_uint(v[3])),
-        "r"(__float_as_uint(v[4])), "r"(__float_as_uint(v[5])), "r"(__float_as_uint(v[6])), "r"(__float_as_uint(v[7])),
-        "r"(__float_as_uint(v[8])), "r"(__float_as_uint(v[9])), "r"(__float_as_uint(v[10])), "r"(__float_as_uint(v[11])),
-        "r"(__float_as_uint(v[12])), "r"(__float_as_uint(v[13])), "r"(__float_as_uint(v[14])), "r"(__float_as_uint(v[15])),
-        "r"(__float_as_uint(v[16])), "r"(__float_as_uint(v[17])), "r"(__float_as_uint(v[18])), "r"(__float_as_uint(v[19])),
-        "r"(__float_as_uint(v[20])), "r"(__float_as_uint(v[21])), "r"(__float_as_uint(v[22])), "r"(__float_as_uint(v[23])),
-        "r"(__float_as_uint(v[24])), "r"(__float_as_uint(v[25])), "r"(__float_as_uint(v[26])), "r"(__float_as_uint(v[27])),
-        "r"(__float_as_uint(v[28])), "r"(__float_as_uint(v[29])), "r"(__float_as_uint(v[30])), "r"(__float_as_uint(v[31]))
-      : "memory");
-  asm volatile("tcgen05.wait::st.sync.aligned;" ::: "memory");
-}
-__device__ __forceinline__ void tmem_st16(uint32_t taddr, const uint32_t* r) {
-  asm volatile(
-      "tcgen05.st.sync.aligned.32x32b.x16.b32 [%0], {%1, %2, %3, %4, %5, %6, %7, %8, %9, %10, %11, %12, %13, %14, %15, %16};"
-      ::"r"(taddr), "r"(r[0]), "r"(r[1]), "r"(r[2]), "r"(r[3]), "r"(r[4]), "r"(r[5]), "r"(r[6]), "r"(r[7]), "r"(r[8]), "r"(r[9]),
-        "r"(r[10]), "r"(r[11]), "r"(r[12]), "r"(r[13]), "r"(r[14]), "r"(r[15])
-      : "memory");
-  asm volatile("tcgen05.wait::st.sync.aligned;" ::: "memory");
-}
-__device__ __forceinline__ void mma_bf16_ts(uint32_t d_tmem, uint32_t a_tmem, uint64_t bdesc, uint32_t idesc, uint32_t accumulate) {
-  asm volatile(
-      "{\n\t.reg .pred p;\n\tsetp.ne.b32 p, %4, 0;\n\t"
-      "tcgen05.mma.cta_group::1.kind::f16 [%0], [%1], %2, %3, p;\n\t}\n"
-      ::"r"(d_tmem), "r"(a_tmem), "l"(bdesc), "r"(idesc), "r"(accumulate)
-      : "memory");
-}
-
-constexpr float AT2_TAU = 8.0f;
-
-__global__ void __launch_bounds__(AT_THREADS, 1)
-attention_tc2_kernel(const __grid_constant__ CUtensorMap tmK, const __grid_constant__ CUtensorMap tmV,
-                     const __grid_constant__ CUtensorMap tmR, const __grid_constant__ AttnP p) {
-  extern __shared__ uint8_t smem_raw[];
-  uint8_t* smem = reinterpret_cast<uint8_t*>((reinterpret_cast<uintptr_t>(smem_raw) + 1023) & ~(uintptr_t)1023);
-  uint8_t* sQ = smem;
-  uint8_t* sX = sQ + AT_Q_BYTES;
-  uint8_t* sKV = sX + 2 * AT_P_BYTES;
-  uint8_t* sLive = sKV + AT_STAGES * AT_STAGE_BYTES;
-  uint64_t* bars = reinterpret_cast<uint64_t*>(sLive + 512);
-  uint64_t* kv_full = bars;
-  uint64_t* kv_empty = kv_full + AT_STAGES;
-  uint64_t* step = kv_empty + AT_STAGES;
-  uint64_t* p_full = step + 2;
-  uint32_t* tmem_slot = reinterpret_cast<uint32_t*>(p_full + 2);
-
-  const int warp = threadIdx.x >> 5, lane = threadIdx.x & 31;
-  const int h = blockIdx.x % p.heads, qt = blockIdx.x / p.heads, b = blockIdx.y;
-  const uint8_t* live = sLive;
-  const int C = p.heads * 32;
-
-  if (warp == 0 && lane == 0) {
-    ptx::prefetch_tmap(&tmK);
-    ptx::prefetch_tmap(&tmV);
-    if (p.has_r) ptx::prefetch_tmap(&tmR);
-    for (int i = 0; i < AT_STAGES; ++i) { ptx::mbar_init(&kv_full[i], 1); ptx::mbar_init(&kv_empty[i], 1); }
-    for (int i = 0; i < 2; ++i) { ptx::mbar_init(&step[i], 1); ptx::mbar_init(&p_full[i], 512); }
-    ptx::fence_mbar_init();
-  }
-  if (warp == 1) {
-    ptx::tmem_alloc(tmem_slot, 512);
-    ptx::tmem_relinquish();
-  }
-  ptx::grid_dep_launch();
-  ptx::grid_dep_wait();
-  {
-    const int q0 = qt * 128, nrows = min(128, p.Q - q0);
-    bool all_live = p.bitmap == nullptr;
-    if (!all_live && p.all_masked)
-      for (int r = lane; r < nrows; r += 32) all_live = all_live || p.all_masked[(long)b * p.Q + q0 + r] != 0;
-    all_live = __any_sync(0xffffffffu, all_live);
-    for (int t = warp; t < p.ntiles; t += AT_THREADS / 32) {
-      bool any = all_live;
-      if (!all_live) {
-        for (int r = lane; r < nrows; r += 32) {
-          const uint32_t* brow = p.bitmap + ((long)b * p.Q + q0 + r) * p.W32;
-#pragma unroll
-          for (int w = 0; w < 4; ++w) {
-            const int widx = t * 4 + w, k0 = t * AT_KT + w * 32;
-            if (widx < p.W32 && k0 < p.K) {
-              const uint32_t valid = (k0 + 32 > p.K) ? ((1u << (p.K - k0)) - 1u) : 0xffffffffu;
-              any = any || ((~__ldg(brow + widx)) & valid) != 0u;
-            }
-          }
-        }
-      }
-      any = __any_sync(0xffffffffu, any);
-      if (lane == 0) sLive[t] = any ? 1 : 0;
-    }
-  }
-  if (warp >= 2 && warp < 6) {
-    const int row = (warp & 3) * 32 + lane, qi = qt * 128 + row;
-    float qv[32];
-    if (qi < p.Q) {
-      const float4* src = reinterpret_cast<const float4*>(p.q + ((long)b * p.Q + qi) * C + h * 32);
-#pragma unroll
-      for (int i = 0; i < 8; ++i) {
-        const float4 x = __ldg(src + i);
-        qv[4 * i] = x.x; qv[4 * i + 1] = x.y; qv[4 * i + 2] = x.z; qv[4 * i + 3] = x.w;
-      }
-    } else {
-#pragma unroll
-      for (int i = 0; i < 32; ++i) qv[i] = 0.f;
-    }
-#pragma unroll
-    for (int c = 0; c < 4; ++c) {
-      uint4 pk;
-      uint32_t* w = reinterpret_cast<uint32_t*>(&pk);
-#pragma unroll
-      for (int j = 0; j < 4; ++j) {
-        __nv_bfloat162 v2 = __floats2bfloat162_rn(qv[8 * c + 2 * j], qv[8 * c + 2 * j + 1]);
-        w[j] = *reinterpret_cast<uint32_t*>(&v2);
-      }
-      *reinterpret_cast<uint4*>(sQ + (row >> 3) * 512 + c * 128 + (row & 7) * 16) = pk;
-    }
-    fence_async_smem();
-  }
-  ptx::tc_fence_before();
-  __syncthreads();
-  ptx::tc_fence_after();
-  const uint32_t tmem_base = *tmem_slot;
-  const uint32_t tmem_S = tmem_base;
-  const uint32_t tmem_P = tmem_base + 256;
-  const uint32_t tmem_O = tmem_base + 384;
-
-  if (warp == 0) {
-    if (lane == 0) {
-      int it = 0;
-      for (int t = next_live(live, 0, p.ntiles); t < p.ntiles; t = next_live(live, t + 1, p.ntiles), ++it) {
-        const int s = it % AT_STAGES;
-        ptx::mbar_wait(&kv_empty[s], ((uint32_t)(it / AT_STAGES) & 1u) ^ 1u);
-        ptx::mbar_expect_tx(&kv_full[s], (p.has_r ? (p.has_r > 1 ? 4 : 3) : 2) * AT_KV_TILE_BYTES);
-        uint8_t* st = sKV + s * AT_STAGE_BYTES;
-        if (p.has_r) {
-          ptx::tma_load_2d(st + 2 * AT_KV_TILE_BYTES, &tmR, &kv_full[s], p.r_col0 + h * 32, t * AT_KT);
-          if (p.has_r > 1) ptx::tma_load_2d(st + 3 * AT_KV_TILE_BYTES, &tmR, &kv_full[s], p.r_lo_off + p.r_col0 + h * 32, t * AT_KT);
-        }
-        ptx::tma_load_3d(st, &tmK, &kv_full[s], h * 32, t * AT_KT, b);
-        ptx::tma_load_3d(st + AT_KV_TILE_BYTES, &tmV, &kv_full[s], h * 32, t * AT_KT, b);
-      }
+      }
+      uint32_t* sm = sMask + s * (AT_MASK_BYTES / 4);
+#pragma unroll
+      for (int c = 0; c < 4; ++c) {
+        const int k0 = t * AT_KT + c * 32;
+        const uint32_t tail = (k0 + 32 <= p.K) ? 0u : (k0 >= p.K) ? 0xffffffffu : ~((1u << (p.K - k0)) - 1u);
+#pragma unroll
+        for (int i = 0; i < 4; ++i) sm[c * 128 + lane + 32 * i] = w[i][c] | tail;
+      }
+      ptx::mbar_arrive(&kv_full[s]);
     }
   } else if (warp == 1) {
     const uint32_t idesc_s = ptx::umma_idesc_bf16(128, AT_KT, false, false);
@@ -563,301 +337,6 @@
     };
     auto issue_qk = [&](int j) {
       const uint64_t kd = kd0 + (uint64_t)((j % AT_STAGES) * (AT_STAGE_BYTES >> 4));
-      const uint32_t d = tmem_S + (uint32_t)((j & 1) * 128);
-#pragma unroll
-      for (int k = 0; k < 2; ++k) ptx::mma_bf16_ss(d, qd0 + (uint64_t)(k * 16), kd + (uint64_t)(k * 2), idesc_s, k);
-      if (p.has_r) {
-#pragma unroll
-        for (int k = 0; k < 4; ++k)
-          if (k < 2 || p.has_r > 1)
-            ptx::mma_bf16_ss(d, qd0 + (uint64_t)((k & 1) * 16),
-                             kd + (uint64_t)((((2 + (k >> 1)) * AT_KV_TILE_BYTES) >> 4) + (k & 1) * 2), idesc_s, 1u);
-      }
-    };
-    for (int j = 0; j < 2 && j < n_live; ++j) {
-      wait_kv(j);
-      if (ptx::elect_one()) { issue_qk(j); ptx::mma_commit(&step[j]); }
-      __syncwarp();
-    }
-    for (int j = 0; j < n_live; ++j) {
-      const int s = j % AT_STAGES;
-      ptx::mbar_wait(&p_full[j & 1], (uint32_t)(j >> 1) & 1u);
-      if (lane == 0) AT_TRACE(j, 0);
-      if (j + 2 < n_live) wait_kv(j + 2);
-      ptx::tc_fence_after();
-      if (lane == 0) AT_TRACE(j, 1);
-      if (ptx::elect_one()) {
-        const uint64_t vd = vd0 + (uint64_t)(s * (AT_STAGE_BYTES >> 4));
-        const uint32_t pa = tmem_P + (uint32_t)((j & 1) * 64);
-#pragma unroll
-        for (int cq = 0; cq < 4; ++cq) {
-          if (p.dbg & 2) break;
-#pragma unroll
-          for (int k = 0; k < 2; ++k)
-            mma_bf16_ts(tmem_O + (uint32_t)(cq * 32), pa + (uint32_t)(cq * 16 + k * 8),
-                        vd + (uint64_t)((cq * 2048 + k * 1024) >> 4), idesc_o, (j > 0 || k > 0) ? 1u : 0u);
-        }
-        if (j + 2 < n_live) issue_qk(j + 2);
-        ptx::mma_commit(&step[j & 1]);
-      }
-      __syncwarp();
-      if (lane == 0) AT_TRACE(j, 2);
-    }
-  } else {
-    const int quarter = warp & 3;
-    const int cq = (warp - 2) >> 2;
-    const int row = quarter * 32 + lane, qi = qt * 128 + row;
-    const bool row_ok = qi < p.Q;
-    const uint32_t lane_off = (uint32_t)(quarter * 32) << 16;
-    const bool ignore_mask = !row_ok || p.bitmap == nullptr || (p.all_masked && p.all_masked[(long)b * p.Q + qi]);
-    const uint32_t* brow = p.bitmap ? p.bitmap + ((long)b * p.Q + (row_ok ? qi : 0)) * p.W32 : nullptr;
-    const uint32_t taddr_o = tmem_O + (uint32_t)(cq * 32) + lane_off;
-    float m_ref = -INFINITY, l_run = 0.f;
-    auto load_mask = [&](int t) -> uint32_t {
-      const int widx = t * 4 + cq;
-      uint32_t word = 0u;
-      if (!ignore_mask && widx < p.W32) word = __ldg(brow + widx);
-      const int k0 = t * AT_KT + cq * 32;
-      if (k0 + 32 > p.K) word |= (k0 >= p.K) ? 0xffffffffu : ~((1u << (p.K - k0)) - 1u);
-      return word;
-    };
-    int it = 0;
-    uint32_t mw_next = 0u;
-    {
-      const int t0 = next_live(live, 0, p.ntiles);
-      if (t0 < p.ntiles) mw_next = load_mask(t0);
-    }
-    for (int t = next_live(live, 0, p.ntiles); t < p.ntiles; ++it) {
-      const int buf = it & 1;
-      const int t_next = next_live(live, t + 1, p.ntiles);
-      const uint32_t mw = mw_next;
-      if (t_next < p.ntiles) mw_next = load_mask(t_next);
-      ptx::mbar_wait(&step[buf], (uint32_t)(it >> 1) & 1u);
-      ptx::tc_fence_after();
-      AT_TRACE_W(it, 3);
-      float v[32];
-      tmem_ld32(tmem_S + (uint32_t)(buf * 128 + cq * 32) + lane_off, v);
-      AT_TRACE_W(it, 4);
-      float mx = -INFINITY;
-#pragma unroll
-      for (int i = 0; i < 32; ++i) {
-        if ((mw >> i) & 1u) v[i] = -INFINITY;
-        mx = fmaxf(mx, v[i]);
-      }
-      mx *= LOG2E;
-      const bool move = mx > m_ref + AT2_TAU;
-      const bool fix = move && m_ref != -INFINITY;
-      if (__any_sync(0xffffffffu, fix)) {
-        ptx::mbar_wait(&step[(it - 1) & 1], (uint32_t)(((it - 1) >> 1) + 1) & 1u);
-        ptx::tc_fence_after();
-        const float sc = fix ? fast_exp2(m_ref - mx) : 1.f;
-        float ov[32];
-        tmem_ld32(taddr_o, ov);
-#pragma unroll
-        for (int i = 0; i < 32; ++i) ov[i] *= sc;
-        tmem_st32(taddr_o, ov);
-        l_run *= sc;
-      }
-      if (move) m_ref = mx;
-      AT_TRACE_W(it, 5);
-      const float mneg = (m_ref == -INFINITY) ? 0.f : -m_ref;
-      uint32_t pk[16];
-      float psum = 0.f;
-#pragma unroll
-      for (int j = 0; j < 16; ++j) {
-        float e0, e1;
-        if (p.dbg & 4) { e0 = fmaf(v[2 * j], LOG2E, mneg); e1 = fmaf(v[2 * j + 1], LOG2E, mneg); }
-        else { e0 = fast_exp2(fmaf(v[2 * j], LOG2E, mneg)); e1 = fast_exp2(fmaf(v[2 * j + 1], LOG2E, mneg)); }
-        __nv_bfloat162 v2 = __floats2bfloat162_rn(e0, e1);
-        pk[j] = *reinterpret_cast<uint32_t*>(&v2);
-        psum += e0 + e1;
-      }
-      l_run += psum;
-      AT_TRACE_W(it, 6);
-      tmem_st16(tmem_P + (uint32_t)(buf * 64 + cq * 16) + lane_off, pk);
-      ptx::tc_fence_before();
-      ptx::mbar_arrive(&p_full[buf]);
-      AT_TRACE_W(it, 7);
-      if (it > 0 && warp == 2) {
-        ptx::mbar_wait(&step[(it - 1) & 1], (uint32_t)(((it - 1) >> 1) + 1) & 1u);
-        if (lane == 0) ptx::mbar_arrive(&kv_empty[(it - 1) % AT_STAGES]);
-      }
-      t = t_next;
-    }
-    float o[32];
-    if (it > 0) {
-      ptx::mbar_wait(&step[(it - 1) & 1], (uint32_t)(((it - 1) >> 1) + 1) & 1u);
-      ptx::tc_fence_after();
-      tmem_ld32(taddr_o, o);
-    } else {
-#pragma unroll
-      for (int i = 0; i < 32; ++i) o[i] = 0.f;
-    }
-    float* xch = reinterpret_cast<float*>(sX);
-    if (cq > 0) {
-      float* dst = xch + ((cq - 1) * 128 + row) * 35;
-      dst[0] = m_ref;
-      dst[1] = l_run;
-#pragma unroll
-      for (int i = 0; i < 32; ++i) dst[2 + i] = o[i];
-    }
-    asm volatile("bar.sync 1, 512;" ::: "memory");
-    if (cq == 0) {
-      float m = m_ref;
-#pragma unroll
-      for (int c2 = 0; c2 < 3; ++c2) m = fmaxf(m, xch[(c2 * 128 + row) * 35]);
-      const float a0 = (m_ref == -INFINITY) ? 0.f : fast_exp2(m_ref - m);
-      l_run *= a0;
-#pragma unroll
-      for (int i = 0; i < 32; ++i) o[i] = (m_ref == -INFINITY) ? 0.f : o[i] * a0;
-#pragma unroll
-      for (int c2 = 0; c2 < 3; ++c2) {
-        const float* src = xch + (c2 * 128 + row) * 35;
-        const float m1 = src[0];
-        if (m1 != -INFINITY) {
-          const float a1 = fast_exp2(m1 - m);
-          l_run += src[1] * a1;
-#pragma unroll
-          for (int i = 0; i < 32; ++i) o[i] += src[2 + i] * a1;
-        }
-      }
-      if (row_ok) store_attn_out(p, b, qi, h, C, o, l_run > 0.f ? 1.0f / l_run : 0.f);
-    }
-  }
-  ptx::tc_fence_before();
-  __syncthreads();
-  if (warp == 1) {
-    __syncwarp();
-    ptx::tmem_dealloc(tmem_base, 512);
-  }
-}
-
-constexpr int AT3_STAGES = 6;
-
-__global__ void __launch_bounds__(AT_THREADS, 1)
-attention_tc3_kernel(const __grid_constant__ CUtensorMap tmK, const __grid_constant__ CUtensorMap tmV,
-                     const __grid_constant__ CUtensorMap tmR, const __grid_constant__ AttnP p) {
-  extern __shared__ uint8_t smem_raw[];
-  uint8_t* smem = reinterpret_cast<uint8_t*>((reinterpret_cast<uintptr_t>(smem_raw) + 1023) & ~(uintptr_t)1023);
-  uint8_t* sQ = smem;
-  uint8_t* sKV = sQ + AT_Q_BYTES;
-  uint8_t* sX = sKV;
-  uint8_t* sLive = sKV + AT3_STAGES * AT_STAGE_BYTES;
-  uint64_t* bars = reinterpret_cast<uint64_t*>(sLive + 512);
-  uint64_t* kv_full = bars;
-  uint64_t* kv_empty = kv_full + AT3_STAGES;
-  uint64_t* step = kv_empty + AT3_STAGES;
-  uint64_t* p_full = step + 3;
-  uint32_t* tmem_slot = reinterpret_cast<uint32_t*>(p_full + 3);
-
-  const int warp = threadIdx.x >> 5, lane = threadIdx.x & 31;
-  const int h = blockIdx.x % p.heads, qt = blockIdx.x / p.heads, b = blockIdx.y;
-  const uint8_t* live = sLive;
-  const int C = p.heads * 32;
-
-  if (warp == 0 && lane == 0) {
-    ptx::prefetch_tmap(&tmK);
-    ptx::prefetch_tmap(&tmV);
-    if (p.has_r) ptx::prefetch_tmap(&tmR);
-    for (int i = 0; i < AT3_STAGES; ++i) { ptx::mbar_init(&kv_full[i], 1); ptx::mbar_init(&kv_empty[i], 1); }
-    for (int i = 0; i < 3; ++i) { ptx::mbar_init(&step[i], 1); ptx::mbar_init(&p_full[i], 512); }
-    ptx::fence_mbar_init();
-  }
-  if (warp == 1) {
-    ptx::tmem_alloc(tmem_slot, 512);
-    ptx::tmem_relinquish();
-  }
-  ptx::grid_dep_launch();
-  ptx::grid_dep_wait();
-  {
-    const int q0 = qt * 128, nrows = min(128, p.Q - q0);
-    bool all_live = p.bitmap == nullptr;
-    if (!all_live && p.all_masked)
-      for (int r = lane; r < nrows; r += 32) all_live = all_live || p.all_masked[(long)b * p.Q + q0 + r] != 0;
-    all_live = __any_sync(0xffffffffu, all_live);
-    for (int t = warp; t < p.ntiles; t += AT_THREADS / 32) {
-      bool any = all_live;
-      if (!all_live) {
-        for (int r = lane; r < nrows; r += 32) {
-          const uint32_t* brow = p.bitmap + ((long)b * p.Q + q0 + r) * p.W32;
-#pragma unroll
-          for (int w = 0; w < 4; ++w) {
-            const int widx = t * 4 + w, k0 = t * AT_KT + w * 32;
-            if (widx < p.W32 && k0 < p.K) {
-              const uint32_t valid = (k0 + 32 > p.K) ? ((1u << (p.K - k0)) - 1u) : 0xffffffffu;
-              any = any || ((~__ldg(brow + widx)) & valid) != 0u;
-            }
-          }
-        }
-      }
-      any = __any_sync(0xffffffffu, any);
-      if (lane == 0) sLive[t] = any ? 1 : 0;
-    }
-  }
-  if (warp >= 2 && warp < 6) {
-    const int row = (warp & 3) * 32 + lane, qi = qt * 128 + row;
-    float qv[32];
-    if (qi < p.Q) {
-      const float4* src = reinterpret_cast<const float4*>(p.q + ((long)b * p.Q + qi) * C + h * 32);
-#pragma unroll
-      for (int i = 0; i < 8; ++i) {
-        const float4 x = __ldg(src + i);
-        qv[4 * i] = x.x; qv[4 * i + 1] = x.y; qv[4 * i + 2] = x.z; qv[4 * i + 3] = x.w;
-      }
-    } else {
-#pragma unroll
-      for (int i = 0; i < 32; ++i) qv[i] = 0.f;
-    }
-#pragma unroll
-    for (int c = 0; c < 4; ++c) {
-      uint4 pk;
-      uint32_t* w = reinterpret_cast<uint32_t*>(&pk);
-#pragma unroll
-      for (int j = 0; j < 4; ++j) {
-        __nv_bfloat162 v2 = __floats2bfloat162_rn(qv[8 * c + 2 * j], qv[8 * c + 2 * j + 1]);
-        w[j] = *reinterpret_cast<uint32_t*>(&v2);
-      }
-      *reinterpret_cast<uint4*>(sQ + (row >> 3) * 512 + c * 128 + (row & 7) * 16) = pk;
-    }
-    fence_async_smem();
-  }
-  ptx::tc_fence_before();
-  __syncthreads();
-  ptx::tc_fence_after();
-  const uint32_t tmem_base = *tmem_slot;
-  const uint32_t tmem_S = tmem_base;
-  const uint32_t tmem_O = tmem_base + 384;
-
-  if (warp == 0) {
-    if (lane == 0) {
-      int it = 0;
-      for (int t = next_live(live, 0, p.ntiles); t < p.ntiles; t = next_live(live, t + 1, p.ntiles), ++it) {
-        const int s = it % AT3_STAGES;
-        ptx::mbar_wait(&kv_empty[s], ((uint32_t)(it / AT3_STAGES) & 1u) ^ 1u);
-        ptx::mbar_expect_tx(&kv_full[s], (p.has_r ? (p.has_r > 1 ? 4 : 3) : 2) * AT_KV_TILE_BYTES);
-        uint8_t* st = sKV + s * AT_STAGE_BYTES;
-        if (p.has_r) {
-          ptx::tma_load_2d(st + 2 * AT_KV_TILE_BYTES, &tmR, &kv_full[s], p.r_col0 + h * 32, t * AT_KT);
-          if (p.has_r > 1) ptx::tma_load_2d(st + 3 * AT_KV_TILE_BYTES, &tmR, &kv_full[s], p.r_lo_off + p.r_col0 + h * 32, t * AT_KT);
-        }
-        ptx::tma_load_3d(st, &tmK, &kv_full[s], h * 32, t * AT_KT, b);
-        ptx::tma_load_3d(st + AT_KV_TILE_BYTES, &tmV, &kv_full[s], h * 32, t * AT_KT, b);
-      }
-    }
-  } else if (warp == 1) {
-    const uint32_t idesc_s = ptx::umma_idesc_bf16(128, AT_KT, false, false);
-    const uint32_t idesc_o = ptx::umma_idesc_bf16(128, 32, false, true);
-    int n_live = 0;
-    for (int t = 0; t < p.ntiles; ++t) n_live += live[t] ? 1 : 0;
-    const uint64_t qd0 = umma_desc(ptx::smem_u32(sQ), 128, 512, 0);
-    const uint64_t kd0 = umma_desc(ptx::smem_u32(sKV), 16, 512, 4);
-    const uint64_t vd0 = umma_desc(ptx::smem_u32(sKV + AT_KV_TILE_BYTES), 1024, 512, 4);
-    auto wait_kv = [&](int j) {
-      ptx::mbar_wait(&kv_full[j % AT3_STAGES], (uint32_t)(j / AT3_STAGES) & 1u);
-      ptx::tc_fence_after();
-    };
-    auto issue_qk = [&](int j) {
-      const uint64_t kd = kd0 + (uint64_t)((j % AT3_STAGES) * (AT_STAGE_BYTES >> 4));
       const uint32_t d = tmem_S + (uint32_t)((j % 3) * 128);
 #pragma unroll
       for (int k = 0; k < 2; ++k) ptx::mma_bf16_ss(d, qd0 + (uint64_t)(k * 16), kd + (uint64_t)(k * 2), idesc_s, k);
@@ -875,7 +354,7 @@
       __syncwarp();
     }
     for (int j = 0; j < n_live; ++j) {
-      const int s = j % AT3_STAGES;
+      const int s = j % AT_STAGES;
       ptx::mbar_wait(&p_full[j % 3], (uint32_t)(j / 3) & 1u);
       if (lane == 0) AT_TRACE(j, 0);
       if (j + 3 < n_live) wait_kv(j + 3);
@@ -886,7 +365,6 @@
         const uint32_t pa = tmem_S + (uint32_t)((j % 3) * 128);
 #pragma unroll
         for (int cq = 0; cq < 4; ++cq) {
-          if (p.dbg & 2) break;
 #pragma unroll
           for (int k = 0; k < 2; ++k)
             mma_bf16_ts(tmem_O + (uint32_t)(cq * 32), pa + (uint32_t)(cq * 32 + k * 8),
@@ -904,78 +382,78 @@
     const int row = quarter * 32 + lane, qi = qt * 128 + row;
     const bool row_ok = qi < p.Q;
     const uint32_t lane_off = (uint32_t)(quarter * 32) << 16;
-    const bool ignore_mask = !row_ok || p.bitmap == nullptr || (p.all_masked && p.all_masked[(long)b * p.Q + qi]);
-    const uint32_t* brow = p.bitmap ? p.bitmap + ((long)b * p.Q + (row_ok ? qi : 0)) * p.W32 : nullptr;
     const uint32_t taddr_o = tmem_O + (uint32_t)(cq * 32) + lane_off;
+    const uint32_t* mrow = sMask + cq * 128 + row;
     float m_ref = -INFINITY, l_run = 0.f;
-    auto load_mask = [&](int t) -> uint32_t {
-      const int widx = t * 4 + cq;
-      uint32_t word = 0u;
-      if (!ignore_mask && widx < p.W32) word = __ldg(brow + widx);
-      const int k0 = t * AT_KT + cq * 32;
-      if (k0 + 32 > p.K) word |= (k0 >= p.K) ? 0xffffffffu : ~((1u << (p.K - k0)) - 1u);
-      return word;
-    };
     int it = 0;
-    uint32_t mw_next = 0u;
-    {
-      const int t0 = next_live(live, 0, p.ntiles);
-      if (t0 < p.ntiles) mw_next = load_mask(t0);
-    }
     for (int t = next_live(live, 0, p.ntiles); t < p.ntiles; ++it) {
-      const int buf = it % 3;
+      const int buf = it % 3, s = it % AT_STAGES;
       const int t_next = next_live(live, t + 1, p.ntiles);
-      const uint32_t mw = mw_next;
-      if (t_next < p.ntiles) mw_next = load_mask(t_next);
+      ptx::mbar_wait(&kv_full[s], (uint32_t)(it / AT_STAGES) & 1u);
+      const uint32_t mw = mrow[s * (AT_MASK_BYTES / 4)];
       ptx::mbar_wait(&step[buf], (uint32_t)(it / 3) & 1u);
       ptx::tc_fence_after();
       AT_TRACE_W(it, 3);
+      uint32_t sv[32];
+      tmem_ld32_issue(tmem_S + (uint32_t)(buf * 128 + cq * 32) + lane_off, sv);
+      tmem_ld32_wait(sv);
+      AT_TRACE_W(it, 4);
       float v[32];
-      tmem_ld32(tmem_S + (uint32_t)(buf * 128 + cq * 32) + lane_off, v);
-      AT_TRACE_W(it, 4);
-      float mx = -INFINITY;
-#pragma unroll
-      for (int i = 0; i < 32; ++i) {
-        if ((mw >> i) & 1u) v[i] = -INFINITY;
-        mx = fmaxf(mx, v[i]);
-      }
-      mx *= LOG2E;
-      const bool move = mx > m_ref + AT2_TAU;
+#pragma unroll
+      for (int i = 0; i < 32; ++i) v[i] = ((mw >> i) & 1u) ? -INFINITY : __uint_as_float(sv[i]);
+      float mt[16];
+#pragma unroll
+      for (int i = 0; i < 16; ++i) mt[i] = fmaxf(v[i], v[i + 16]);
+#pragma unroll
+      for (int n = 8; n > 0; n >>= 1)
+#pragma unroll
+        for (int i = 0; i < n; ++i) mt[i] = fmaxf(mt[i], mt[i + n]);
+      const float mx = mt[0] * LOG2E;
+      const bool move = mx > m_ref + AT_TAU;
       const bool fix = move && m_ref != -INFINITY;
       if (__any_sync(0xffffffffu, fix)) {
         ptx::mbar_wait(&step[(it - 1) % 3], (uint32_t)(((it - 1) / 3) + 1) & 1u);
         ptx::tc_fence_after();
         const float sc = fix ? fast_exp2(m_ref - mx) : 1.f;
-        float ov[32];
-        tmem_ld32(taddr_o, ov);
-#pragma unroll
-        for (int i = 0; i < 32; ++i) ov[i] *= sc;
-        tmem_st32(taddr_o, ov);
+#pragma unroll
+        for (int hf = 0; hf < 2; ++hf) {
+          float ov[16];
+          uint32_t ou[16];
+          ptx::tmem_ld16(taddr_o + (uint32_t)(hf * 16), ov);
+#pragma unroll
+          for (int i = 0; i < 16; ++i) ou[i] = __float_as_uint(ov[i] * sc);
+          tmem_st16_issue(taddr_o + (uint32_t)(hf * 16), ou);
+          tmem_st16_wait(ou);
+        }
         l_run *= sc;
       }
       if (move) m_ref = mx;
       AT_TRACE_W(it, 5);
       const float mneg = (m_ref == -INFINITY) ? 0.f : -m_ref;
       uint32_t pk[16];
-      float psum = 0.f;
+      float2 e[16];
 #pragma unroll
       for (int j = 0; j < 16; ++j) {
-        float e0, e1;
-        if (p.dbg & 4) { e0 = fmaf(v[2 * j], LOG2E, mneg); e1 = fmaf(v[2 * j + 1], LOG2E, mneg); }
-        else { e0 = fast_exp2(fmaf(v[2 * j], LOG2E, mneg)); e1 = fast_exp2(fmaf(v[2 * j + 1], LOG2E, mneg)); }
-        __nv_bfloat162 v2 = __floats2bfloat162_rn(e0, e1);
+        e[j] = fma2(make_float2(v[2 * j], v[2 * j + 1]), make_float2(LOG2E, LOG2E), make_float2(mneg, mneg));
+        e[j].x = fast_exp2(e[j].x);
+        e[j].y = fast_exp2(e[j].y);
+        __nv_bfloat162 v2 = __floats2bfloat162_rn(e[j].x, e[j].y);
         pk[j] = *reinterpret_cast<uint32_t*>(&v2);
-        psum += e0 + e1;
-      }
-      l_run += psum;
+      }
+      tmem_st16_issue(tmem_S + (uint32_t)(buf * 128 + cq * 32) + lane_off, pk);
+#pragma unroll
+      for (int n = 8; n > 0; n >>= 1)
+#pragma unroll
+        for (int j = 0; j < n; ++j) e[j] = add2(e[j], e[j + n]);
+      l_run += e[0].x + e[0].y;
       AT_TRACE_W(it, 6);
-      tmem_st16(tmem_S + (uint32_t)(buf * 128 + cq * 32) + lane_off, pk);
+      tmem_st16_wait(pk);
       ptx::tc_fence_before();
       ptx::mbar_arrive(&p_full[buf]);
       AT_TRACE_W(it, 7);
       if (it > 0 && warp == 2) {
         ptx::mbar_wait(&step[(it - 1) % 3], (uint32_t)(((it - 1) / 3) + 1) & 1u);
-        if (lane == 0) ptx::mbar_arrive(&kv_empty[(it - 1) % AT3_STAGES]);
+        if (lane == 0) ptx::mbar_arrive(&kv_empty[(it - 1) % AT_STAGES]);
       }
       t = t_next;
     }
@@ -1017,7 +495,9 @@
           for (int i = 0; i < 32; ++i) o[i] += src[2 + i] * a1;
         }
       }
-      if (row_ok) store_attn_out(p, b, qi, h, C, o, l_run > 0.f ? 1.0f / l_run : 0.f);
+      if (row_ok)
+        store_attn_out(p, blockIdx.y, (blockIdx.x / p.heads) * 128 + row, blockIdx.x % p.heads, p.heads * 32, o,
+                       l_run > 0.f ? 1.0f / l_run : 0.f);
     }
   }
   ptx::tc_fence_before();
@@ -1049,6 +529,7 @@
                  cudaStream_t s, const void* r_table, long r_cols, int r_col0, int out_mode) {
   const int Q = t->cfg.num_queries, heads = t->cfg.num_heads, C = t->cfg.embed_dim;
   const int ntiles = (num_keys + AT_KT - 1) / AT_KT, nqt = (Q + 127) / 128;
+  if (ntiles > AT_MAX_TILES) return tc_fail(t, CGG_ERR_BAD_SHAPE, "more than 512 key tiles");
   CUtensorMap mK, mV;
   int st = make_map_kv(t, &mK, k, num_keys, kv_stride, kv_bstride, batch, C);
   if (st != CGG_OK) return st;
@@ -1072,36 +553,29 @@
   p.has_r = r_table ? 2 : 0;
   p.r_col0 = r_col0; p.r_lo_off = (int)(r_cols / 2);
   p.out_hl = out_mode;
-#ifdef CGG_AT_TRACING
-  static const int at_dbg = getenv("CGG_AT_DBG") ? atoi(getenv("CGG_AT_DBG")) : 0;
-  p.dbg = at_dbg;
-  if (at_dbg & 1) p.has_r = 0;
-#else
-  p.dbg = 0;
-#endif
-  if (ntiles > 512) return tc_fail(t, CGG_ERR_BAD_SHAPE, "more than 512 key tiles");
-  const size_t smem = 1024 + AT_Q_BYTES + 2 * AT_P_BYTES + AT_STAGES * AT_STAGE_BYTES + 512 + (2 * AT_STAGES + 4) * 8 + 16;
+  if (bitmap) {
+    if ((size_t)batch * nqt * ntiles > t->live_bytes) return tc_fail(t, CGG_ERR_BAD_SHAPE, "live-tile flags exceed their buffer");
+    TCU(launch_pdl(attention_live_kernel, dim3(nqt, batch), dim3(512), 0, s, bitmap, all_masked, Q, num_keys, W32, ntiles,
+                   nqt, t->live_buf));
+    count_launch();
+    TCU(cudaGetLastError());
+    p.live = t->live_buf;
+  }
   if (!t->attn_attr_set) {
-    TCU(cudaFuncSetAttribute(attention_tc_kernel, cudaFuncAttributeMaxDynamicSharedMemorySize, (int)smem));
-    TCU(cudaFuncSetAttribute(attention_tc2_kernel, cudaFuncAttributeMaxDynamicSharedMemorySize, (int)smem));
-    TCU(cudaFuncSetAttribute(attention_tc3_kernel, cudaFuncAttributeMaxDynamicSharedMemorySize, 227 * 1024));
+    TCU(cudaFuncSetAttribute(masked_attention_tc_kernel, cudaFuncAttributeMaxDynamicSharedMemorySize, (int)AT_SMEM));
     t->attn_attr_set = true;
   }
   static const bool trace = getenv("CGG_AT_TRACE") != nullptr;
   p.trace = trace ? atoi(getenv("CGG_AT_TRACE")) : 0;
-  static const int use_v1 = getenv("CGG_ATTN_V1") ? atoi(getenv("CGG_ATTN_V1")) : 0;
-  static const int use_v3 = getenv("CGG_ATTN_V3") ? atoi(getenv("CGG_ATTN_V3")) : 1;
-  const size_t smem3 = 1024 + AT_Q_BYTES + AT3_STAGES * AT_STAGE_BYTES + 512 + (2 * AT3_STAGES + 6) * 8 + 16;
-  if (use_v1) TCU(launch_pdl(attention_tc_kernel, dim3(heads * nqt, batch), dim3(AT_THREADS), smem, s, mK, mV, mR, p));
-  else if (use_v3) TCU(launch_pdl(attention_tc3_kernel, dim3(heads * nqt, batch), dim3(AT_THREADS), smem3, s, mK, mV, mR, p));
-  else TCU(launch_pdl(attention_tc2_kernel, dim3(heads * nqt, batch), dim3(AT_THREADS), smem, s, mK, mV, mR, p));
+  TCU(launch_pdl(masked_attention_tc_kernel, dim3(heads * nqt, batch), dim3(AT_THREADS), AT_SMEM, s, mK, mV, mR, p));
   count_launch();
   TCU(cudaGetLastError());
   if (trace && ntiles >= 24) {
     cudaStreamSynchronize(s);
     long long tr[64];
     cudaMemcpyFromSymbol(tr, g_at_trace, sizeof(tr));
-    fprintf(stderr, "[attention trace] K=%d cycles rel. to tile 16: mma(P ready, PV committed, QK(j+2) committed) softmax(S ready, S loaded, P arrived, O(j-1) ready, folded)\n", num_keys);
+    fprintf(stderr, "[attention trace] K=%d cycles rel. to tile 16: mma(P ready, K/V(j+3) ready, PV+QK(j+3) committed) "
+                    "softmax(mask read, S loaded, rescaled, P issued, P arrived)\n", num_keys);
     for (int i = 0; i < 8; ++i) {
       fprintf(stderr, "  j=%d:", 16 + i);
       for (int j = 0; j < 8; ++j) fprintf(stderr, " %7lld", tr[i * 8 + j] - tr[0]);
```
